# NVIDIA-Merlin/distributed-embeddings

Hardware: NVIDIA H100
Metric: DLRM global samples/sec (device-timed, max over ranks) (higher is better)
Workload: dtype bf16

## Files before the change

distributed_embeddings_b200/models/dlrm_fast.py:

```python
from __future__ import annotations

import os
from typing import Optional

import torch
from torch import nn

from ..ops import _native
from ..parallel.comm import CommContext
from ..parallel.fused import FusedEngine
from ..utils import nvtx
from ..utils.lr_schedule import LearningRateScheduler
from .dlrm import DLRM


def _pad8(n: int) -> int:
  return (n + 7) // 8 * 8


class _Layer:

  def __init__(self, lin: nn.Linear, relu: bool):
    self.lin = lin
    self.relu = relu
    self.out_f, self.in_f = lin.weight.shape
    self.in_pad = _pad8(self.in_f)
    self.w_off = self.b_off = 0
    self.w_numel = self.out_f * self.in_pad
    self.b_numel = _pad8(self.out_f)


class DLRMTrainStep:

  def __init__(self, model: DLRM, lr: float = 24.0, embedding_optimizer: str = "sgd",
               scheduler: Optional[LearningRateScheduler] = None, use_cuda_graph: bool = True,
               embedding_optimizer_kwargs: Optional[dict] = None, overlap: bool = True,
               gemm: str = "cublas"):
    if gemm not in ("cublas", "fused_dgrad", "tcgen05", "tcgen05_pair"):
      raise ValueError("gemm must be cublas | fused_dgrad | tcgen05 | tcgen05_pair")
    self.gemm = gemm
    self.model = model
    self.emb = model.embedding
    if self.emb.backend != "fused":
      raise ValueError("DLRMTrainStep needs the fused embedding back end")
    self.dev = self.emb.device
    self.ops = _native.require()
    self.world = self.emb.world_size
    self.ctx = CommContext.for_group(self.emb.group, self.dev)
    self.scheduler = scheduler
    self.use_cuda_graph = use_cuda_graph
    self.overlap = overlap
    self.emb.set_optimizer(embedding_optimizer, lr=lr, **(embedding_optimizer_kwargs or {}))
    if self.emb._engine is None:
      self.emb._engine = FusedEngine(self.emb)
    self.engine: FusedEngine = self.emb._engine
    self.n_emb = len(model.table_sizes)
    self.dim = model.embedding_dim
    sp_env = os.environ.get("DE_B200_STREAM_PUSH", "auto")
    self._stream_push = self.world > 1 and (sp_env == "1" or (sp_env == "auto" and self.world >= 4))
    self._push_stream = torch.cuda.Stream(device=self.dev) if self._stream_push else None
    self._push_ready = torch.cuda.Event() if self._stream_push else None

    lins_b = [m for m in model.bottom_mlp.net if isinstance(m, nn.Linear)]
    lins_t = [m for m in model.top_mlp.net if isinstance(m, nn.Linear)]
    self.bottom = [_Layer(l, True) for l in lins_b]
    self.top = [_Layer(l, True) for l in lins_t[:-1]]
    self.head = _Layer(lins_t[-1], False)
    if self.head.out_f != 1:
      raise ValueError("the top MLP must end in a single logit")
    layers = self.bottom + self.top + [self.head]
    self._dp_slots = []
    pos = 0
    if len(self.emb.dp_layers):
      if embedding_optimizer != "sgd":
        raise ValueError("replicated tables in the fast step are updated by the dense SGD "
                         "kernel: use embedding_optimizer='sgd' or data_parallel_threshold=None")
      for layer in self.emb.dp_layers:
        w = layer.embeddings
        self._dp_slots.append((pos, tuple(w.shape)))
        pos += _pad8(w.numel())
    for L in layers:
      L.w_off = pos
      pos += L.w_numel
      L.b_off = pos
      pos += L.b_numel
    self.n_flat = pos
    dev = self.dev
    self.p32 = torch.zeros(pos, dtype=torch.float32, device=dev)
    self.p16 = torch.zeros(pos, dtype=torch.bfloat16, device=dev)
    if self.world > 1:
      self.gsym = self.ctx.alloc_multicast(pos * 4, "dense_grads") or \
          self.ctx.alloc(pos * 4, "dense_grads")
      self.allreduce_kind = "nvls_multimem" if getattr(self.gsym, "mc_ptr", 0) else "p2p"
      self.g32 = self.gsym.view(torch.float32, (pos,))
    else:
      self.gsym = None
      self.allreduce_kind = "none"
      self.g32 = torch.zeros(pos, dtype=torch.float32, device=dev)
    with torch.no_grad():
      dp_targets = []
      for layer, (off, shape) in zip(self.emb.dp_layers, self._dp_slots):
        n = shape[0] * shape[1]
        view = self.p32[off:off + n].view(shape)
        view.copy_(layer.embeddings.data)
        layer.embeddings.data = view
        dp_targets.append(self.g32[off:off + n].view(shape))
      if self._dp_slots:
        self.engine.set_dp_grad_targets(dp_targets)
        self.engine._tables_dirty = True
        self.engine._key = None
      for L in layers:
        wv = self.p32[L.w_off:L.w_off + L.w_numel].view(L.out_f, L.in_pad)
        wv[:, :L.in_f].copy_(L.lin.weight)
        L.lin.weight.data = wv[:, :L.in_f]
        bv = self.p32[L.b_off:L.b_off + L.out_f]
        bv.copy_(L.lin.bias)
        L.lin.bias.data = bv
        L.w16 = self.p16[L.w_off:L.w_off + L.w_numel].view(L.out_f, L.in_pad)
        L.b16 = self.p16[L.b_off:L.b_off + L.out_f]
        L.gw = self.g32[L.w_off:L.w_off + L.w_numel].view(L.out_f, L.in_pad)
        L.gb = self.g32[L.b_off:L.b_off + L.b_numel]
        L.w16T = torch.empty(L.in_pad, L.out_f, dtype=torch.bfloat16, device=dev)
      self.p16.copy_(self.p32)
      self._refresh_transposes()
    self.lr_t = torch.full((1,), float(lr), dtype=torch.float32, device=dev)
    self.engine.share_lr(self.lr_t)
    self.lr = float(lr)
    self.loss = torch.zeros(1, dtype=torch.float32, device=dev)
    self._batch = None
    self._graph = None
    self._side = torch.cuda.Stream(device=dev) if overlap else None
    self._wgrad_overlap = os.environ.get("DE_B200_WGRAD_STREAM", "auto")
    self._wstream = torch.cuda.Stream(device=dev) if overlap else None
    ar_env = os.environ.get("DE_B200_AR_OVERLAP", "auto")
    ar_on = ar_env == "1" or (ar_env == "auto" and self.world >= 4)
    self._ar_stream = torch.cuda.Stream(device=dev) if (overlap and self.world > 1 and ar_on) \
        else None

  def _refresh_transposes(self):
    if self.gemm == "cublas":
      return
    for L in self.bottom[1:] + self.top[1:]:
      L.w16T.copy_(L.w16.t())

  def _linear_fwd(self, L, x):
    if self.gemm in ("tcgen05", "tcgen05_pair"):
      pair = self.gemm == "tcgen05_pair" and L.out_f >= 256
      self.ops.gemm_tn_bias_act(x, L.w16, L.b16, L.y, True, 512 if pair else 0)
    else:
      torch._addmm_activation(L.b16, x, L.w16.t(), out=L.y)
    return L.y

  def _wgrad(self, L, x):
    use = self._wstream is not None and (
        self._wgrad_overlap == "1" or
        (self._wgrad_overlap == "auto" and (self._batch or 0) >= 49152))
    if not use:
      torch.mm(L.dy.t(), x, out_dtype=torch.float32, out=L.gw)
      return
    self._w_used = True
    self._wstream.wait_stream(torch.cuda.current_stream())
    with torch.cuda.stream(self._wstream):
      torch.mm(L.dy.t(), x, out_dtype=torch.float32, out=L.gw)

  def _dgrad_relu(self, L, x_below, dx, gb_below):
    if self.gemm == "cublas":
      torch.mm(L.dy, L.w16, out=dx)
      self.ops.relu_bwd_bias(dx, x_below, gb_below)
    else:
      self.ops.gemm_dgrad_relu_bias(L.dy, L.w16T, x_below, dx, gb_below, 0)

  def _alloc(self, b: int):
    dev, bf = self.dev, torch.bfloat16
    if self._stream_push:
      self.engine.enable_streamed_push(max(1024, -(-b // 16)))
    self.engine.prepare(b, [1] * self.n_emb, ids64=False)
    self.cat_stage = self.engine.in_flat[:self.n_emb * b].view(self.n_emb, b)
    self.num_in = torch.zeros(b, self.bottom[0].in_f, dtype=torch.float32, device=dev)
    self.lab_in = torch.zeros(b, dtype=torch.float32, device=dev)
    self.x0 = torch.zeros(b, self.bottom[0].in_pad, dtype=bf, device=dev)
    for L in self.bottom + self.top:
      L.y = torch.empty(b, L.out_f, dtype=bf, device=dev)
      L.dy = torch.empty(b, L.out_f, dtype=bf, device=dev)
    self.z = torch.zeros(b, self.top[0].in_pad, dtype=bf, device=dev)
    self.dz = torch.empty(b, self.top[0].in_pad, dtype=bf, device=dev)
    self._batch = b
    self._graph = None
    self._stage = [(torch.zeros_like(self.cat_stage), torch.zeros_like(self.num_in),
                    torch.zeros_like(self.lab_in)) for _ in range(2)]
    self._slot_dev = torch.zeros(1, dtype=torch.int32, device=dev)
    self._slot_host = torch.tensor([[0], [1]], dtype=torch.int32).pin_memory()
    self._h2d_done = [torch.cuda.Event(), torch.cuda.Event()]
    self._consumed = [torch.cuda.Event(), torch.cuda.Event()]
    self._prefetched = 0
    self._consumed_n = 0
    self._use_stage = False

  def _forward(self):
    ops = self.ops
    if self._use_stage:
      a, b_ = self._stage
      ops.select_copy([a[0], a[1], a[2]], [b_[0], b_[1], b_[2]],
                      [self.cat_stage, self.num_in, self.lab_in], self._slot_dev)
    eng = self.engine
    if self._side is not None:
      self._side.wait_stream(torch.cuda.current_stream())
      with torch.cuda.stream(self._side):
        eng.launch_forward()
    ops.cast_pad(self.num_in, self.x0)
    x = self.x0
    for L in self.bottom:
      x = self._linear_fwd(L, x)
    if self._side is not None:
      torch.cuda.current_stream().wait_stream(self._side)
    else:
      eng.launch_forward()
    if eng.out_needs_reduce:
      eng.wait_output()
      ops.interact_fwd(x, eng.out, self.n_emb, self.z, [])
    else:
      ops.interact_fwd(x, eng.out, self.n_emb, self.z, eng.sync_out_wait())
    x = self.z
    for L in self.top:
      x = self._linear_fwd(L, x)

  def _backward(self):
    ops, eng = self.ops, self.engine
    b = self._batch
    last = self.top[-1]
    self.loss.zero_()
    H = self.head
    ops.head_loss(last.y, H.w16.view(-1), H.b16, self.lab_in, 1.0 / b, last.dy,
                  H.gw.view(-1), H.gb, last.gb, self.loss, None)
    for i in range(len(self.top) - 1, -1, -1):
      L = self.top[i]
      x = self.top[i - 1].y if i > 0 else self.z
      dx = self.top[i - 1].dy if i > 0 else self.dz
      self._wgrad(L, x)
      if i > 0:
        self._dgrad_relu(L, x, dx, self.top[i - 1].gb)
      else:
        torch.mm(L.dy, L.w16, out=dx)
    if self._ar_stream is not None:
      ar = self._ar_stream
      ar.wait_stream(torch.cuda.current_stream())
      if getattr(self, "_w_used", False):
        ar.wait_stream(self._wstream)
      off = self.top[0].w_off
      with torch.cuda.stream(ar):
        self.ctx.allreduce_(self.gsym, self.n_flat - off, torch.float32, scale=1.0 / self.world,
                            byte_offset=off * 4, max_blocks=32)
    hb = self.bottom[-1]
    pushed = eng.streamed_push
    if pushed:
      eng.push_counters.zero_()
      self._push_ready.record(torch.cuda.current_stream())
      ops.interact_bwd(hb.y, eng.out, self.n_emb, self.dz, hb.dy, 0, 0, 1.0, eng.routes_stage,
                       len(eng.routes_stage_np), [], eng.push_counters, eng.push_chunk_rows)
      self._push_stream.wait_event(self._push_ready)
      with torch.cuda.stream(self._push_stream):
        eng.launch_streamed_push()
    else:
      ops.interact_bwd(hb.y, eng.out, self.n_emb, self.dz, hb.dy, 0, 0, 1.0, eng.routes_all,
                       len(eng.routes_all_np), eng.sync_grad_signal(), None, 0)
    if self._side is not None:
      self._side.wait_stream(torch.cuda.current_stream())
      if pushed:
        self._side.wait_stream(self._push_stream)
      with torch.cuda.stream(self._side):
        eng.backward_inplace()
    else:
      if pushed:
        torch.cuda.current_stream().wait_stream(self._push_stream)
      eng.backward_inplace()
    ops.relu_bwd_bias(hb.dy, hb.y, hb.gb)
    for i in range(len(self.bottom) - 1, -1, -1):
      L = self.bottom[i]
      x = self.bottom[i - 1].y if i > 0 else self.x0
      self._wgrad(L, x)
      if i > 0:
        self._dgrad_relu(L, x, self.bottom[i - 1].dy, self.bottom[i - 1].gb)
    if self._dp_slots and self._side is not None:
      torch.cuda.current_stream().wait_stream(self._side)
    if getattr(self, "_w_used", False):
      torch.cuda.current_stream().wait_stream(self._wstream)
      self._w_used = False
    if self.world > 1:
      if self._ar_stream is not None:
        ar = self._ar_stream
        ar.wait_stream(torch.cuda.current_stream())
        with torch.cuda.stream(ar):
          self.ctx.allreduce_(self.gsym, self.top[0].w_off, torch.float32, scale=1.0 / self.world)
        torch.cuda.current_stream().wait_stream(ar)
      else:
        self.ctx.allreduce_(self.gsym, self.n_flat, torch.float32, scale=1.0 / self.world)
    ops.dense_sgd(self.p32, self.p16, self.g32, self.lr_t, 1.0)
    self._refresh_transposes()
    if self._side is not None:
      torch.cuda.current_stream().wait_stream(self._side)

  def _step_impl(self):
    with nvtx.range("dlrm_forward"):
      self._forward()
    with nvtx.range("dlrm_backward_update"):
      self._backward()

  def set_lr(self, lr: float):
    self.lr = float(lr)
    self.lr_t.fill_(self.lr)
    if self.emb._fused_optimizer is not None:
      self.emb._fused_optimizer["lr"] = self.lr

  def load_batch(self, numerical, categorical, labels):
    b = int(numerical.shape[0])
    if b != self._batch:
      self._alloc(b)
    self.num_in.copy_(numerical, non_blocking=True)
    self.lab_in.copy_(labels.reshape(-1), non_blocking=True)
    if isinstance(categorical, (list, tuple)):
      for v, c in zip(self.engine.in_views, categorical):
        v.copy_(c.reshape(v.shape), non_blocking=True)
    else:
      self.cat_stage.copy_(categorical, non_blocking=True)

  def prefetch(self, numerical, categorical, labels):
    b = int(numerical.shape[0])
    if b != self._batch:
      self._alloc(b)
    if not self._use_stage:
      self._use_stage = True
      self._graph = None
      self._copy_stream = torch.cuda.Stream(device=self.dev)
    slot = self._prefetched & 1
    cs = self._copy_stream
    if self._prefetched >= 2:
      cs.wait_event(self._consumed[slot])
    with torch.cuda.stream(cs):
      st = self._stage[slot]
      st[0].copy_(categorical, non_blocking=True)
      st[1].copy_(numerical, non_blocking=True)
      st[2].copy_(labels.reshape(-1), non_blocking=True)
      self._h2d_done[slot].record(cs)
    self._prefetched += 1

  def run_prefetched(self) -> torch.Tensor:
    assert self._consumed_n < self._prefetched, "call prefetch() first"
    slot = self._consumed_n & 1
    main = torch.cuda.current_stream()
    main.wait_event(self._h2d_done[slot])
    self._slot_dev.copy_(self._slot_host[slot], non_blocking=True)
    loss = self.run()
    self._consumed[slot].record(main)
    self._consumed_n += 1
    return loss

  def run(self) -> torch.Tensor:
    if self.scheduler is not None:
      self.set_lr(self.scheduler.step())
    if not self.use_cuda_graph:
      self._step_impl()
      return self.loss
    if self._graph is None:
      self.lr_t.zero_()
      self.engine.dry_updates(True)
      s = torch.cuda.Stream(device=self.dev)
      s.wait_stream(torch.cuda.current_stream())
      with torch.cuda.stream(s):
        for _ in range(2):
          self._step_impl()
      torch.cuda.current_stream().wait_stream(s)
      torch.cuda.synchronize()
      self.engine.dry_updates(False)
      g = torch.cuda.CUDAGraph()
      with torch.cuda.graph(g):
        self._step_impl()
      self._graph = g
      self.set_lr(self.lr)
    self._graph.replay()
    return self.loss

  def step(self, numerical, categorical, labels) -> torch.Tensor:
    self.load_batch(numerical, categorical, labels)
    return self.run()
```

distributed_embeddings_b200/ops/csrc/bindings.cpp:

```cpp
#include <ATen/cuda/CUDAContext.h>
#include <c10/cuda/CUDAGuard.h>
#include <c10/cuda/CUDAStream.h>
#include <cuda_runtime.h>
#include <torch/library.h>
#include <torch/torch.h>

#include <cstdlib>
#include <cstring>
#include <mutex>
#include <string>
#include <unordered_map>
#include <vector>

#include "de_b200.h"

namespace {

using at::Tensor;

#define DE_CUDA_CHECK(expr)                                                              \
  do {                                                                                   \
    cudaError_t _e = (expr);                                                             \
    TORCH_CHECK(_e == cudaSuccess, "CUDA error in " #expr ": ", cudaGetErrorString(_e)); \
  } while (0)

cudaStream_t cur_stream() { return at::cuda::getCurrentCUDAStream().stream(); }

int sm_count() {
  static int cached = -1;
  if (cached < 0) cached = at::cuda::getCurrentDeviceProperties()->multiProcessorCount;
  return cached;
}

de::PeerPtrs to_peers(at::IntArrayRef ptrs) {
  TORCH_CHECK(ptrs.size() <= de::kMaxPeers, "at most ", de::kMaxPeers, " peers are supported");
  de::PeerPtrs p;
  std::memset(&p, 0, sizeof(p));
  for (size_t i = 0; i < ptrs.size(); ++i) p.p[i] = reinterpret_cast<void*>(ptrs[i]);
  return p;
}

void check_launch() {
  cudaError_t e = cudaGetLastError();
  TORCH_CHECK(e == cudaSuccess, "kernel launch failed: ", cudaGetErrorString(e));
}

struct SyncCtx {
  de::PeerPtrs flags;
  uint32_t* state;
  int* error_flag;
  unsigned long long timeout;
  int rank, world;
};
std::vector<SyncCtx>& sync_ctxs() {
  static std::vector<SyncCtx> v;
  return v;
}
std::mutex& sync_mutex() {
  static std::mutex m;
  return m;
}

int64_t sync_ctx_create(at::IntArrayRef flag_ptrs, Tensor state, int64_t rank, int64_t world,
                        int64_t timeout_cycles, int64_t error_ptr) {
  TORCH_CHECK(state.is_cuda() && state.scalar_type() == at::kInt && state.is_contiguous() &&
                  state.numel() >= de::kSyncStateWords,
              "sync state must be an int32 CUDA tensor of >= ", de::kSyncStateWords, " words");
  SyncCtx c;
  c.flags = to_peers(flag_ptrs);
  c.state = reinterpret_cast<uint32_t*>(state.data_ptr<int>());
  c.error_flag = reinterpret_cast<int*>(error_ptr);
  c.timeout = static_cast<unsigned long long>(timeout_cycles);
  c.rank = static_cast<int>(rank);
  c.world = static_cast<int>(world);
  std::lock_guard<std::mutex> lock(sync_mutex());
  sync_ctxs().push_back(c);
  return static_cast<int64_t>(sync_ctxs().size()) - 1;
}

de::SyncArgs to_sync(at::IntArrayRef spec) {
  de::SyncArgs a = de::no_sync();
  if (spec.size() == 0) return a;
  TORCH_CHECK(spec.size() == 5, "sync spec = {handle, wait_ch, wait_abs_ch, signal_ch, slot}");
  SyncCtx c;
  {
    std::lock_guard<std::mutex> lock(sync_mutex());
    TORCH_CHECK(spec[0] >= 0 && spec[0] < static_cast<int64_t>(sync_ctxs().size()),
                "unknown sync context");
    c = sync_ctxs()[spec[0]];
  }
  for (int i = 1; i <= 3; ++i)
    TORCH_CHECK(spec[i] >= -1 && spec[i] < de::kSyncChannels, "sync channel out of range");
  TORCH_CHECK(spec[4] >= 0 && spec[4] < 2 * de::kSyncChannels, "sync counter slot out of range");
  a.flags = c.flags;
  a.state = c.state;
  a.error_flag = c.error_flag;
  a.timeout = c.timeout;
  a.rank = c.rank;
  a.world = c.world;
  a.wait_ch = static_cast<int32_t>(spec[1]);
  a.wait_abs_ch = static_cast<int32_t>(spec[2]);
  a.signal_ch = static_cast<int32_t>(spec[3]);
  a.counter_slot = static_cast<int32_t>(spec[4]);
  return a;
}

int dtype_code(at::ScalarType t) {
  if (t == at::kFloat) return 0;
  if (t == at::kBFloat16) return 1;
  if (t == at::kHalf) return 2;
  TORCH_CHECK(false, "activations / gradients must be fp32, bf16 or fp16");
  return -1;
}

void sync_only(at::IntArrayRef sync) {
  de::launch_sync_only(to_sync(sync), cur_stream());
  check_launch();
}

std::vector<int64_t> struct_sizes() {
  return {static_cast<int64_t>(sizeof(de::InputDesc)), static_cast<int64_t>(sizeof(de::TableDesc)),
          static_cast<int64_t>(de::kMaxPeers), static_cast<int64_t>(sizeof(de::GradRoute)),
          static_cast<int64_t>(de::kSyncStateWords)};
}

void lookup_fwd(const Tensor& descs, int64_t n_inputs, int64_t batch, int64_t src_batch,
                int64_t dst_batch, int64_t dst_stride, at::IntArrayRef src_ptrs,
                at::IntArrayRef dst_ptrs, int64_t rot, bool ids64, int64_t act_dtype, bool vec4,
                at::IntArrayRef sync, int64_t tile_samples, int64_t table_dtype, bool vec8) {
  TORCH_CHECK(descs.is_cuda(), "descs must live on the GPU");
  TORCH_CHECK(table_dtype >= 0 && table_dtype <= 2, "table_dtype: 0 fp32, 1 bf16, 2 fp16");
  c10::cuda::CUDAGuard guard(descs.device());
  de::launch_lookup_fwd(reinterpret_cast<const de::InputDesc*>(descs.data_ptr()),
                        static_cast<int>(n_inputs), batch, src_batch, dst_batch, dst_stride,
                        to_peers(src_ptrs), to_peers(dst_ptrs), static_cast<int>(rot), ids64,
                        static_cast<int>(act_dtype), vec4, sm_count(), cur_stream(),
                        to_sync(sync), static_cast<int>(tile_samples),
                        static_cast<int>(table_dtype), vec8);
  check_launch();
}

void scatter_add_bwd(const Tensor& descs, int64_t n_inputs, int64_t batch, int64_t src_batch,
                     int64_t grad_batch, int64_t grad_stride, at::IntArrayRef src_ptrs,
                     at::IntArrayRef grad_ptrs, int64_t rot, double scale, int64_t scale_ptr,
                     bool ids64, int64_t act_dtype, bool vec4, bool vec8, at::IntArrayRef sync,
                     bool staged) {
  TORCH_CHECK(descs.is_cuda(), "descs must live on the GPU");
  c10::cuda::CUDAGuard guard(descs.device());
  de::launch_scatter_add_bwd(reinterpret_cast<const de::InputDesc*>(descs.data_ptr()),
                             static_cast<int>(n_inputs), batch, src_batch, grad_batch, grad_stride,
                             to_peers(src_ptrs), to_peers(grad_ptrs), static_cast<int>(rot),
                             static_cast<float>(scale), reinterpret_cast<const float*>(scale_ptr),
                             ids64, static_cast<int>(act_dtype), vec4, sm_count(), cur_stream(),
                             vec8, to_sync(sync), staged);
  check_launch();
}

int bit_length(int64_t v) {
  int b = 0;
  while (v > 0) {
    ++b;
    v >>= 1;
  }
  return b < 1 ? 1 : b;
}

bool use_own_sort() {
  static const bool own = [] {
    const char* v = std::getenv("DE_B200_SORT");
    return !(v != nullptr && std::string(v) == "cub");
  }();
  return own;
}

std::tuple<Tensor, Tensor> radix_sort_pairs(const Tensor& keys, const Tensor& items,
                                            int64_t end_bit) {
  TORCH_CHECK(keys.is_cuda() && keys.scalar_type() == at::kLong && keys.is_contiguous());
  TORCH_CHECK(items.is_cuda() && items.scalar_type() == at::kInt && items.is_contiguous() &&
              items.numel() == keys.numel());
  c10::cuda::CUDAGuard guard(keys.device());
  const int64_t n = keys.numel();
  TORCH_CHECK(n < (int64_t(1) << 31), "own radix sort: too many items");
  Tensor ka = keys.clone(), ia = items.clone();
  Tensor kb = at::empty_like(ka), ib = at::empty_like(ia);
  if (n == 0) return {ka, ia};
  Tensor temp = at::empty({static_cast<int64_t>(de::radix_sort_temp_bytes(n))},
                          at::TensorOptions().device(keys.device()).dtype(at::kByte));
  int where = de::radix_sort_pairs(temp.data_ptr(), ka.data_ptr<int64_t>(),
                                   reinterpret_cast<uint32_t*>(ia.data_ptr<int>()),
                                   kb.data_ptr<int64_t>(),
                                   reinterpret_cast<uint32_t*>(ib.data_ptr<int>()), n,
                                   static_cast<int>(end_bit), cur_stream());
  check_launch();
  if (where == 0) return {ka, ia};
  return {kb, ib};
}

std::tuple<Tensor, Tensor> radix_sort_pairs32(const Tensor& keys, const Tensor& items,
                                              int64_t end_bit) {
  TORCH_CHECK(keys.is_cuda() && keys.scalar_type() == at::kInt && keys.is_contiguous());
  TORCH_CHECK(items.is_cuda() && items.scalar_type() == at::kInt && items.is_contiguous() &&
              items.numel() == keys.numel());
  c10::cuda::CUDAGuard guard(keys.device());
  const int64_t n = keys.numel();
  TORCH_CHECK(n < (int64_t(1) << 31), "own radix sort: too many items");
  Tensor ka = keys.clone(), ia = items.clone();
  Tensor kb = at::empty_like(ka), ib = at::empty_like(ia);
  Tensor out = at::empty({n}, keys.options().dtype(at::kLong));
  if (n == 0) return {out, ia};
  Tensor temp = at::empty({static_cast<int64_t>(de::radix_sort_temp_bytes(n))},
                          at::TensorOptions().device(keys.device()).dtype(at::kByte));
  int where = de::radix_sort_pairs32(
      temp.data_ptr(), reinterpret_cast<uint32_t*>(ka.data_ptr<int>()),
      reinterpret_cast<uint32_t*>(ia.data_ptr<int>()),
      reinterpret_cast<uint32_t*>(kb.data_ptr<int>()),
      reinterpret_cast<uint32_t*>(ib.data_ptr<int>()), out.data_ptr<int64_t>(), n,
      static_cast<int>(end_bit), cur_stream());
  check_launch();
  return {out, where == 0 ? ia : ib};
}

std::tuple<Tensor, Tensor> head_segments(const Tensor& sorted_keys) {
  TORCH_CHECK(sorted_keys.is_cuda() && sorted_keys.scalar_type() == at::kLong &&
              sorted_keys.is_contiguous());
  c10::cuda::CUDAGuard guard(sorted_keys.device());
  const int64_t n = sorted_keys.numel();
  auto i64 = at::TensorOptions().device(sorted_keys.device()).dtype(at::kLong);
  Tensor seg_start = at::empty({n + 1}, i64);
  Tensor n_unique = at::zeros({1}, i64);
  if (n == 0) return {seg_start, n_unique};
  Tensor temp = at::empty({static_cast<int64_t>(de::head_segments_temp_bytes(n))},
                          at::TensorOptions().device(sorted_keys.device()).dtype(at::kByte));
  de::head_segments(temp.data_ptr(), sorted_keys.data_ptr<int64_t>(), n,
                    seg_start.data_ptr<int64_t>(), n_unique.data_ptr<int64_t>(), cur_stream());
  check_launch();
  return {seg_start, n_unique};
}

std::tuple<Tensor, Tensor, Tensor, Tensor> sort_items(const Tensor& descs, const Tensor& tables,
                                                      int64_t n_tables, int64_t n_inputs,
                                                      int64_t batch, int64_t src_batch,
                                                      at::IntArrayRef src_ptrs, bool ids64,
                                                      int64_t n_items, int64_t total_rows,
                                                      bool prefill_sentinel) {
  TORCH_CHECK(descs.is_cuda() && tables.is_cuda());
  TORCH_CHECK(n_inputs * batch < (int64_t(1) << 32),
              "sorted update: n_inputs * batch = ", n_inputs * batch, " does not fit 32-bit items");
  c10::cuda::CUDAGuard guard(descs.device());
  auto stream = cur_stream();
  auto i64 = at::TensorOptions().device(descs.device()).dtype(at::kLong);
  auto i32 = at::TensorOptions().device(descs.device()).dtype(at::kInt);
  Tensor keys = prefill_sentinel ? at::full({n_items}, total_rows, i64) : at::empty({n_items}, i64);
  Tensor keys_sorted = at::empty({n_items}, i64);
  Tensor items = at::empty({n_items}, i32), items_sorted = at::empty({n_items}, i32);
  Tensor seg_start = at::empty({n_items + 1}, i64);
  Tensor n_unique = at::zeros({1}, i64);
  if (n_items == 0) return {keys_sorted, items_sorted, seg_start, n_unique};
  if (use_own_sort() && total_rows < (int64_t(1) << 32) - 1) {
    TORCH_CHECK(n_items < (int64_t(1) << 31), "own radix sort: too many items");
    Tensor k32a = prefill_sentinel
                      ? at::full({n_items}, static_cast<int64_t>(static_cast<int32_t>(
                                                static_cast<uint32_t>(total_rows))), i32)
                      : at::empty({n_items}, i32);
    Tensor k32b = at::empty({n_items}, i32);
    de::launch_build_keys(reinterpret_cast<const de::InputDesc*>(descs.data_ptr()),
                          reinterpret_cast<const de::TableDesc*>(tables.data_ptr()),
                          static_cast<int>(n_tables), static_cast<int>(n_inputs), batch,
                          src_batch, to_peers(src_ptrs), ids64, k32a.data_ptr(),
                          reinterpret_cast<uint32_t*>(items.data_ptr<int>()), sm_count(), stream,
                          true);
    check_launch();
    size_t sort_bytes = de::radix_sort_temp_bytes(n_items);
    size_t head_bytes = de::head_segments_temp_bytes(n_items);
    Tensor temp = at::empty({static_cast<int64_t>(std::max(sort_bytes, head_bytes))},
                            at::TensorOptions().device(descs.device()).dtype(at::kByte));
    int where = de::radix_sort_pairs32(
        temp.data_ptr(), reinterpret_cast<uint32_t*>(k32a.data_ptr<int>()),
        reinterpret_cast<uint32_t*>(items.data_ptr<int>()),
        reinterpret_cast<uint32_t*>(k32b.data_ptr<int>()),
        reinterpret_cast<uint32_t*>(items_sorted.data_ptr<int>()),
        keys_sorted.data_ptr<int64_t>(), n_items, bit_length(total_rows), stream);
    if (where == 0) std::swap(items, items_sorted);
    de::head_segments(temp.data_ptr(), keys_sorted.data_ptr<int64_t>(), n_items,
                      seg_start.data_ptr<int64_t>(), n_unique.data_ptr<int64_t>(), stream);
    check_launch();
    return {keys_sorted, items_sorted, seg_start, n_unique};
  }
  de::launch_build_keys(reinterpret_cast<const de::InputDesc*>(descs.data_ptr()),
                        reinterpret_cast<const de::TableDesc*>(tables.data_ptr()),
                        static_cast<int>(n_tables), static_cast<int>(n_inputs), batch, src_batch,
                        to_peers(src_ptrs), ids64, keys.data_ptr<int64_t>(),
                        reinterpret_cast<uint32_t*>(items.data_ptr<int>()), sm_count(), stream);
  check_launch();
  if (use_own_sort()) {
    TORCH_CHECK(n_items < (int64_t(1) << 31), "own radix sort: too many items");
    size_t sort_bytes = de::radix_sort_temp_bytes(n_items);
    size_t head_bytes = de::head_segments_temp_bytes(n_items);
    Tensor temp = at::empty({static_cast<int64_t>(std::max(sort_bytes, head_bytes))},
                            at::TensorOptions().device(descs.device()).dtype(at::kByte));
    int where = de::radix_sort_pairs(temp.data_ptr(), keys.data_ptr<int64_t>(),
                                     reinterpret_cast<uint32_t*>(items.data_ptr<int>()),
                                     keys_sorted.data_ptr<int64_t>(),
                                     reinterpret_cast<uint32_t*>(items_sorted.data_ptr<int>()),
                                     n_items, bit_length(total_rows), stream);
    if (where == 0) {
      std::swap(keys, keys_sorted);
      std::swap(items, items_sorted);
    }
    de::head_segments(temp.data_ptr(), keys_sorted.data_ptr<int64_t>(), n_items,
                      seg_start.data_ptr<int64_t>(), n_unique.data_ptr<int64_t>(), stream);
    check_launch();
    return {keys_sorted, items_sorted, seg_start, n_unique};
  }
  size_t sort_bytes = de::sort_pairs_temp_bytes(n_items);
  size_t uniq_bytes = de::unique_temp_bytes(n_items);
  Tensor temp = at::empty({static_cast<int64_t>(std::max(sort_bytes, uniq_bytes)) + 16},
                          at::TensorOptions().device(descs.device()).dtype(at::kByte));
  de::sort_pairs(temp.data_ptr(), sort_bytes, keys.data_ptr<int64_t>(),
                 keys_sorted.data_ptr<int64_t>(),
                 reinterpret_cast<const uint32_t*>(items.data_ptr<int>()),
                 reinterpret_cast<uint32_t*>(items_sorted.data_ptr<int>()), n_items,
                 bit_length(total_rows), stream);
  de::unique_segments(temp.data_ptr(), uniq_bytes, keys_sorted.data_ptr<int64_t>(), n_items,
                      seg_start.data_ptr<int64_t>(), n_unique.data_ptr<int64_t>(), stream);
  check_launch();
  return {keys_sorted, items_sorted, seg_start, n_unique};
}

void segment_update(const Tensor& descs, const Tensor& tables, int64_t n_tables, int64_t batch,
                    int64_t grad_batch, int64_t grad_stride, at::IntArrayRef grad_ptrs,
                    const Tensor& sorted_keys, const Tensor& sorted_items, const Tensor& seg_start,
                    const Tensor& n_unique, int64_t opt_kind, double lr, double eps, double beta1,
                    double beta2, double bias1, double bias2, double grad_scale,
                    double weight_decay, int64_t lr_ptr, const c10::optional<Tensor>& emit_keys,
                    const c10::optional<Tensor>& emit_rows, int64_t max_width, int64_t act_dtype,
                    bool vec4, const c10::optional<Tensor>& scratch, int64_t step_ptr,
                    int64_t table_dtype) {
  c10::cuda::CUDAGuard guard(descs.device());
  TORCH_CHECK(table_dtype >= 0 && table_dtype <= 2, "table_dtype: 0 fp32, 1 bf16, 2 fp16");
  de::OptimizerArgs opt;
  opt.kind = static_cast<int32_t>(opt_kind);
  opt.lr = static_cast<float>(lr);
  opt.eps = static_cast<float>(eps);
  opt.beta1 = static_cast<float>(beta1);
  opt.beta2 = static_cast<float>(beta2);
  opt.bias1 = static_cast<float>(bias1);
  opt.bias2 = static_cast<float>(bias2);
  opt.grad_scale = static_cast<float>(grad_scale);
  opt.weight_decay = static_cast<float>(weight_decay);
  opt.lr_ptr = reinterpret_cast<const float*>(lr_ptr);
  opt.step_ptr = reinterpret_cast<const float*>(step_ptr);
  if (opt.kind == de::kOptEmit) TORCH_CHECK(emit_keys.has_value() && emit_rows.has_value());
  if (scratch.has_value() && vec4 && max_width <= 128 && opt.kind != de::kOptEmit) {
    const int64_t n_items = sorted_keys.numel();
    const int64_t sw = (max_width + 3) / 4 * 4;
    TORCH_CHECK(scratch->scalar_type() == at::kFloat && scratch->is_contiguous() &&
                    scratch->numel() >= ((n_items + 31) / 32) * sw,
                "scratch too small for the balanced update");
    bool ok = de::launch_balanced_update(
        reinterpret_cast<const de::InputDesc*>(descs.data_ptr()),
        reinterpret_cast<const de::TableDesc*>(tables.data_ptr()), static_cast<int>(n_tables),
        batch, grad_batch, grad_stride, to_peers(grad_ptrs), sorted_keys.data_ptr<int64_t>(),
        reinterpret_cast<const uint32_t*>(sorted_items.data_ptr<int>()), n_items,
        seg_start.data_ptr<int64_t>(), n_unique.data_ptr<int64_t>(), opt,
        scratch->data_ptr<float>(), static_cast<int>(sw), static_cast<int>(max_width),
        static_cast<int>(act_dtype), sm_count(), cur_stream(), static_cast<int>(table_dtype));
    TORCH_CHECK(ok, "balanced update launch failed");
    check_launch();
    return;
  }
  de::launch_segment_update(
      reinterpret_cast<const de::InputDesc*>(descs.data_ptr()),
      reinterpret_cast<const de::TableDesc*>(tables.data_ptr()), static_cast<int>(n_tables), batch,
      grad_batch, grad_stride, to_peers(grad_ptrs), sorted_keys.data_ptr<int64_t>(),
      reinterpret_cast<const uint32_t*>(sorted_items.data_ptr<int>()),
      seg_start.data_ptr<int64_t>(), n_unique.data_ptr<int64_t>(), sorted_keys.numel(), opt,
      emit_keys.has_value() ? emit_keys->data_ptr<int64_t>() : nullptr,
      emit_rows.has_value() ? emit_rows->data_ptr<float>() : nullptr, static_cast<int>(max_width),
      static_cast<int>(act_dtype), vec4, sm_count(), cur_stream(), static_cast<int>(table_dtype));
  check_launch();
}

Tensor upload_bytes(const void* host, size_t bytes, const at::Device& dev) {
  Tensor t = at::empty({static_cast<int64_t>(bytes)},
                       at::TensorOptions().device(dev).dtype(at::kByte));
  DE_CUDA_CHECK(cudaMemcpyAsync(t.data_ptr(), host, bytes, cudaMemcpyHostToDevice, cur_stream()));
  return t;
}

de::InputDesc single_desc(const void* table, const Tensor& values,
                          const c10::optional<Tensor>& offsets, int64_t hotness, int64_t rows,
                          int64_t width, int64_t combiner) {
  de::InputDesc d;
  std::memset(&d, 0, sizeof(d));
  d.table = table;
  d.ids = values.data_ptr();
  d.offsets = offsets.has_value() ? offsets->data_ptr<int64_t>() : nullptr;
  d.sub_rows = rows;
  d.width = static_cast<int32_t>(width);
  d.hotness = offsets.has_value() ? 0 : static_cast<int32_t>(hotness);
  d.combiner = static_cast<int32_t>(combiner);
  return d;
}

void check_ids(const Tensor& values, const c10::optional<Tensor>& offsets) {
  TORCH_CHECK(values.is_cuda() && values.is_contiguous(), "ids must be a contiguous CUDA tensor");
  TORCH_CHECK(values.scalar_type() == at::kInt || values.scalar_type() == at::kLong,
              "ids must be int32 or int64");
  if (offsets.has_value())
    TORCH_CHECK(offsets->is_cuda() && offsets->scalar_type() == at::kLong &&
                    offsets->is_contiguous(),
                "row_splits must be a contiguous int64 CUDA tensor");
}

Tensor embedding_lookup_fwd(const Tensor& param, const Tensor& values,
                            const c10::optional<Tensor>& offsets, int64_t hotness, int64_t batch,
                            int64_t combiner, bool out_bf16) {
  const auto pt = param.scalar_type();
  TORCH_CHECK(param.is_cuda() && param.dim() == 2 &&
                  (pt == at::kFloat || pt == at::kBFloat16 || pt == at::kHalf) &&
                  param.is_contiguous(),
              "param must be a contiguous fp32, bf16 or fp16 [rows, width] CUDA tensor");
  check_ids(values, offsets);
  c10::cuda::CUDAGuard guard(param.device());
  const int64_t width = param.size(1);
  const int tdt = dtype_code(pt);
  Tensor out = at::empty({batch, width}, param.options().dtype(out_bf16 ? at::kBFloat16 : pt));
  if (batch == 0) return out;
  de::InputDesc d = single_desc(param.data_ptr(), values, offsets, hotness, param.size(0), width,
                                combiner);
  Tensor dd = upload_bytes(&d, sizeof(d), param.device());
  de::PeerPtrs src, dst;
  std::memset(&src, 0, sizeof(src));
  std::memset(&dst, 0, sizeof(dst));
  dst.p[0] = out.data_ptr();
  const int64_t avg_hot = std::max<int64_t>(1, values.numel() / std::max<int64_t>(batch, 1));
  int64_t lanes_per_row = 1;
  while (lanes_per_row < (width + 3) / 4 && lanes_per_row < 32) lanes_per_row *= 2;
  const int64_t ts = std::max<int64_t>(32 / lanes_per_row, std::min<int64_t>(32, 64 / avg_hot));
  de::launch_lookup_fwd(reinterpret_cast<const de::InputDesc*>(dd.data_ptr()), 1, batch, batch,
                        batch, width, src, dst, 0, values.scalar_type() == at::kLong,
                        out_bf16 ? 1 : tdt, width % 4 == 0, sm_count(), cur_stream(),
                        de::no_sync(), static_cast<int>(std::max<int64_t>(1, ts)), tdt,
                        width % 8 == 0 && reinterpret_cast<uintptr_t>(param.data_ptr()) % 16 == 0);
  check_launch();
  return out;
}

void embedding_scatter_add(Tensor dst, const Tensor& values, const c10::optional<Tensor>& offsets,
                           int64_t hotness, int64_t batch, int64_t combiner, const Tensor& grad,
                           double scale) {
  TORCH_CHECK(dst.is_cuda() && dst.dim() == 2 && dst.scalar_type() == at::kFloat &&
              dst.is_contiguous());
  TORCH_CHECK(grad.is_cuda() && grad.dim() == 2 && grad.stride(1) == 1);
  check_ids(values, offsets);
  if (batch == 0) return;
  c10::cuda::CUDAGuard guard(dst.device());
  const int64_t width = dst.size(1);
  de::InputDesc d = single_desc(dst.data_ptr(), values, offsets, hotness, dst.size(0), width,
                                combiner);
  Tensor dd = upload_bytes(&d, sizeof(d), dst.device());
  de::PeerPtrs src, gp;
  std::memset(&src, 0, sizeof(src));
  std::memset(&gp, 0, sizeof(gp));
  gp.p[0] = grad.data_ptr();
  const int gdt = dtype_code(grad.scalar_type());
  const int64_t gstride = grad.stride(0);
  const bool vec4 = (width % 4 == 0) && (gstride % 4 == 0) &&
                    (reinterpret_cast<uintptr_t>(grad.data_ptr()) % 16 == 0);
  de::launch_scatter_add_bwd(reinterpret_cast<const de::InputDesc*>(dd.data_ptr()), 1, batch,
                             batch, batch, gstride, src, gp, 0, static_cast<float>(scale), nullptr,
                             values.scalar_type() == at::kLong, gdt, vec4, sm_count(),
                             cur_stream(), false, de::no_sync());
  check_launch();
}

std::tuple<Tensor, Tensor> embedding_lookup_grad(const Tensor& values,
                                                 const c10::optional<Tensor>& offsets,
                                                 int64_t hotness, int64_t batch, int64_t combiner,
                                                 const Tensor& grad, int64_t num_rows) {
  TORCH_CHECK(grad.is_cuda() && grad.dim() == 2 && grad.stride(1) == 1);
  check_ids(values, offsets);
  c10::cuda::CUDAGuard guard(grad.device());
  const int64_t width = grad.size(1);
  const int64_t n_items = values.numel();
  auto f32 = grad.options().dtype(at::kFloat);
  auto i64 = grad.options().dtype(at::kLong);
  if (n_items == 0) return {at::empty({0}, i64), at::empty({0, width}, f32)};
  de::InputDesc d = single_desc(nullptr, values, offsets, hotness, num_rows, width, combiner);
  de::TableDesc t;
  std::memset(&t, 0, sizeof(t));
  t.rows = num_rows;
  t.width = static_cast<int32_t>(width);
  Tensor dd = upload_bytes(&d, sizeof(d), grad.device());
  Tensor td = upload_bytes(&t, sizeof(t), grad.device());
  auto sorted = sort_items(dd, td, 1, 1, batch, batch, {}, values.scalar_type() == at::kLong,
                           n_items, num_rows, false);
  Tensor emit_keys = at::empty({n_items}, i64);
  Tensor emit_rows = at::empty({n_items, width}, f32);
  const int gdt = dtype_code(grad.scalar_type());
  const int64_t gstride = grad.stride(0);
  const bool vec4 = (width % 4 == 0) && (gstride % 4 == 0) &&
                    (reinterpret_cast<uintptr_t>(grad.data_ptr()) % 16 == 0);
  std::vector<int64_t> gp = {reinterpret_cast<int64_t>(grad.data_ptr())};
  segment_update(dd, td, 1, batch, batch, gstride, gp, std::get<0>(sorted), std::get<1>(sorted),
                 std::get<2>(sorted), std::get<3>(sorted), de::kOptEmit, 0, 0, 0, 0, 1, 1, 1.0, 0, 0,
                 emit_keys, emit_rows, width, gdt, vec4, c10::nullopt, 0, 0);
  int64_t n_unique = std::get<3>(sorted).item<int64_t>();
  if (n_unique > 0) {
    int64_t last = emit_keys.narrow(0, n_unique - 1, 1).item<int64_t>();
    if (last >= num_rows) --n_unique;
  }
  return {emit_keys.narrow(0, 0, n_unique), emit_rows.narrow(0, 0, n_unique)};
}

Tensor row_to_split(const Tensor& indices, int64_t num_rows) {
  TORCH_CHECK(indices.is_cuda() && indices.dim() == 2 && indices.size(1) == 2 &&
                  indices.scalar_type() == at::kLong && indices.is_contiguous(),
              "indices must be a contiguous int64 [nnz, 2] CUDA tensor");
  c10::cuda::CUDAGuard guard(indices.device());
  Tensor splits = at::empty({num_rows + 1}, indices.options());
  de::launch_row_to_split(indices.data_ptr<int64_t>(), indices.size(0), num_rows,
                          splits.data_ptr<int64_t>(), cur_stream());
  check_launch();
  return splits;
}

void hash_init(Tensor table) {
  TORCH_CHECK(table.is_cuda() && table.scalar_type() == at::kLong && table.is_contiguous());
  c10::cuda::CUDAGuard guard(table.device());
  de::launch_hash_init(table.data_ptr<int64_t>(), table.numel() / 2, cur_stream());
  check_launch();
}

Tensor integer_lookup(Tensor table, Tensor count, Tensor next_index, const Tensor& keys,
                      int64_t capacity) {
  TORCH_CHECK(table.is_cuda() && count.is_cuda() && next_index.is_cuda() && keys.is_cuda());
  TORCH_CHECK(table.scalar_type() == at::kLong && keys.scalar_type() == at::kLong &&
              next_index.scalar_type() == at::kLong && count.scalar_type() == at::kInt);
  c10::cuda::CUDAGuard guard(table.device());
  Tensor k = keys.contiguous();
  Tensor out = at::empty_like(k);
  de::launch_integer_lookup(table.data_ptr<int64_t>(), table.numel() / 2,
                            reinterpret_cast<uint32_t*>(count.data_ptr<int>()),
                            next_index.data_ptr<int64_t>(), k.data_ptr<int64_t>(), k.numel(),
                            capacity, out.data_ptr<int64_t>(), cur_stream());
  check_launch();
  return out;
}

void barrier(at::IntArrayRef flag_ptrs, Tensor epoch, int64_t rank, int64_t world, int64_t channel,
             int64_t timeout_cycles, int64_t error_ptr) {
  c10::cuda::CUDAGuard guard(epoch.device());
  de::launch_barrier(to_peers(flag_ptrs), reinterpret_cast<uint32_t*>(epoch.data_ptr<int>()),
                     static_cast<int>(rank), static_cast<int>(world), static_cast<int>(channel),
                     static_cast<unsigned long long>(timeout_cycles),
                     reinterpret_cast<int*>(error_ptr), cur_stream());
  check_launch();
}

void allreduce(at::IntArrayRef buf_ptrs, at::IntArrayRef flag_ptrs, Tensor epoch, int64_t rank,
               int64_t world, int64_t n_elems, double scale, bool bf16, int64_t channel,
               int64_t timeout_cycles, int64_t error_ptr, int64_t mc_ptr, int64_t max_blocks) {
  c10::cuda::CUDAGuard guard(epoch.device());
  if (mc_ptr != 0) {
    de::launch_allreduce_multimem(reinterpret_cast<void*>(mc_ptr), to_peers(flag_ptrs),
                                  reinterpret_cast<uint32_t*>(epoch.data_ptr<int>()),
                                  static_cast<int>(rank), static_cast<int>(world), n_elems,
                                  static_cast<float>(scale), bf16, static_cast<int>(channel),
                                  static_cast<unsigned long long>(timeout_cycles),
                                  reinterpret_cast<int*>(error_ptr), sm_count(), cur_stream(),
                         static_cast<int>(max_blocks));
  } else {
    de::launch_allreduce(to_peers(buf_ptrs), to_peers(flag_ptrs),
                         reinterpret_cast<uint32_t*>(epoch.data_ptr<int>()),
                         static_cast<int>(rank), static_cast<int>(world), n_elems,
                         static_cast<float>(scale), bf16, static_cast<int>(channel),
                         static_cast<unsigned long long>(timeout_cycles),
                         reinterpret_cast<int*>(error_ptr), sm_count(), cur_stream(),
                         static_cast<int>(max_blocks));
  }
  check_launch();
}

void p2p_store_bench(const Tensor& src, int64_t dst_ptr, int64_t n_rows, int64_t row_bytes,
                     int64_t vec_bytes, int64_t dst_stride, int64_t unroll, int64_t blocks,
                     int64_t threads) {
  TORCH_CHECK(src.is_cuda() && src.is_contiguous() &&
              src.numel() * src.element_size() >= n_rows * row_bytes);
  TORCH_CHECK(row_bytes % vec_bytes == 0 && (vec_bytes == 4 || vec_bytes == 8 || vec_bytes == 16));
  TORCH_CHECK((row_bytes / vec_bytes >= 32 && (row_bytes / vec_bytes) % 32 == 0) ||
              32 % (row_bytes / vec_bytes) == 0);
  TORCH_CHECK(unroll >= 1 && unroll <= 8 && threads % 32 == 0 && threads <= 1024);
  c10::cuda::CUDAGuard guard(src.device());
  de::launch_p2p_store_bench(src.data_ptr(), reinterpret_cast<void*>(dst_ptr), n_rows,
                             static_cast<int>(row_bytes), static_cast<int>(vec_bytes), dst_stride,
                             static_cast<int>(unroll), static_cast<int>(blocks),
                             static_cast<int>(threads), cur_stream());
  check_launch();
}

void push_segments(const Tensor& segs, const Tensor& src, at::IntArrayRef dst_ptrs,
                   int64_t max_seg_elems, at::IntArrayRef sync) {
  TORCH_CHECK(segs.is_cuda() && segs.scalar_type() == at::kLong && segs.is_contiguous() &&
              segs.dim() == 2 && segs.size(1) == 4);
  TORCH_CHECK(src.is_cuda() && src.is_contiguous() &&
              (src.element_size() == 4 || src.element_size() == 8));
  c10::cuda::CUDAGuard guard(src.device());
  de::launch_push_segments(segs.data_ptr<int64_t>(), static_cast<int>(segs.size(0)),
                           src.data_ptr(), to_peers(dst_ptrs),
                           static_cast<int>(src.element_size()), max_seg_elems, sm_count(),
                           cur_stream(), to_sync(sync));
  check_launch();
}

void push_grad(const Tensor& routes, int64_t n_routes, const Tensor& src, int64_t dst_dtype,
               double scale, at::IntArrayRef sync) {
  TORCH_CHECK(routes.is_cuda() && routes.scalar_type() == at::kByte &&
              routes.numel() >= n_routes * static_cast<int64_t>(sizeof(de::GradRoute)));
  TORCH_CHECK(src.is_cuda() && src.dim() == 2 && src.stride(1) == 1);
  c10::cuda::CUDAGuard guard(src.device());
  de::launch_push_grad(reinterpret_cast<const de::GradRoute*>(routes.data_ptr()),
                       static_cast<int>(n_routes), src.data_ptr(), src.stride(0),
                       dtype_code(src.scalar_type()), static_cast<int>(dst_dtype), src.size(0),
                       static_cast<float>(scale), sm_count(), cur_stream(), to_sync(sync));
  check_launch();
}

void stream_push(at::IntArrayRef src_ptrs, at::IntArrayRef dst_ptrs, at::IntArrayRef row_bytes,
                 const Tensor& counters, int64_t chunk_rows, int64_t rows, int64_t blocks,
                 at::IntArrayRef sync) {
  TORCH_CHECK(src_ptrs.size() == dst_ptrs.size() && src_ptrs.size() == row_bytes.size() &&
              src_ptrs.size() <= de::kMaxPeers);
  TORCH_CHECK(counters.is_cuda() && counters.scalar_type() == at::kInt && chunk_rows > 0 &&
              counters.numel() >= (rows + chunk_rows - 1) / chunk_rows);
  de::PushPlan plan;
  std::memset(&plan, 0, sizeof(plan));
  plan.n = static_cast<int32_t>(src_ptrs.size());
  for (size_t i = 0; i < src_ptrs.size(); ++i) {
    TORCH_CHECK(row_bytes[i] % 16 == 0 && src_ptrs[i] % 16 == 0 && dst_ptrs[i] % 16 == 0,
                "streamed push needs 16-byte aligned rows");
    plan.src[i] = reinterpret_cast<const void*>(src_ptrs[i]);
    plan.dst[i] = reinterpret_cast<void*>(dst_ptrs[i]);
    plan.row_bytes[i] = row_bytes[i];
  }
  c10::cuda::CUDAGuard guard(counters.device());
  de::SyncArgs sa = to_sync(sync);
  de::launch_stream_push(plan, reinterpret_cast<const uint32_t*>(counters.data_ptr<int>()),
                         static_cast<int>(chunk_rows), rows, sa.timeout, sa.error_flag,
                         static_cast<int>(blocks), cur_stream(), sa);
  check_launch();
}

void rowslice_reduce(const Tensor& partial, int64_t out_ptr, int64_t out_stride,
                     int64_t out_dtype, const Tensor& cols) {
  TORCH_CHECK(partial.is_cuda() && partial.dim() == 3 && partial.scalar_type() == at::kFloat &&
              partial.is_contiguous());
  TORCH_CHECK(cols.is_cuda() && cols.scalar_type() == at::kInt && cols.is_contiguous() &&
              cols.dim() == 2 && cols.size(1) == 3);
  c10::cuda::CUDAGuard guard(partial.device());
  de::launch_rowslice_reduce(partial.data_ptr<float>(), static_cast<int>(partial.size(0)),
                             partial.size(1), partial.size(2), reinterpret_cast<void*>(out_ptr),
                             out_stride, static_cast<int>(out_dtype), cols.data_ptr<int>(),
                             static_cast<int>(cols.size(0)), cur_stream());
  check_launch();
}

void gather_segments(const Tensor& segs, at::IntArrayRef src_ptrs, Tensor dst,
                     int64_t max_seg_elems) {
  TORCH_CHECK(segs.is_cuda() && segs.scalar_type() == at::kLong && segs.is_contiguous());
  TORCH_CHECK(dst.is_cuda() && dst.is_contiguous());
  c10::cuda::CUDAGuard guard(dst.device());
  de::launch_gather_segments(segs.data_ptr<int64_t>(), static_cast<int>(segs.size(0)),
                             to_peers(src_ptrs), dst.data_ptr(),
                             static_cast<int>(dst.element_size()), max_seg_elems, cur_stream());
  check_launch();
}

void gather_ragged(const Tensor& segs, at::IntArrayRef val_ptrs, at::IntArrayRef split_ptrs,
                   Tensor dst_vals, Tensor goff, int64_t b, int64_t max_cap) {
  TORCH_CHECK(segs.is_cuda() && segs.scalar_type() == at::kLong && segs.is_contiguous());
  TORCH_CHECK(goff.is_cuda() && goff.scalar_type() == at::kLong && dst_vals.is_cuda());
  c10::cuda::CUDAGuard guard(dst_vals.device());
  de::launch_gather_ragged(segs.data_ptr<int64_t>(), static_cast<int>(segs.size(0)),
                           to_peers(val_ptrs), to_peers(split_ptrs), dst_vals.data_ptr(),
                           goff.data_ptr<int64_t>(), b, static_cast<int>(val_ptrs.size()),
                           static_cast<int>(dst_vals.element_size()), max_cap, cur_stream());
  check_launch();
}

void select_copy(at::TensorList src0, at::TensorList src1, at::TensorList dst,
                 const Tensor& slot_flag) {
  TORCH_CHECK(src0.size() == dst.size() && src1.size() == dst.size() && dst.size() <= 4);
  TORCH_CHECK(slot_flag.is_cuda() && slot_flag.scalar_type() == at::kInt);
  const void* s0[4];
  const void* s1[4];
  void* d[4];
  int64_t nb[4];
  for (size_t i = 0; i < dst.size(); ++i) {
    TORCH_CHECK(src0[i].is_contiguous() && src1[i].is_contiguous() && dst[i].is_contiguous());
    nb[i] = dst[i].numel() * dst[i].element_size();
    TORCH_CHECK(src0[i].numel() * src0[i].element_size() == nb[i] &&
                src1[i].numel() * src1[i].element_size() == nb[i] && nb[i] % 16 == 0,
                "select_copy segments must match and be multiples of 16 bytes");
    s0[i] = src0[i].data_ptr();
    s1[i] = src1[i].data_ptr();
    d[i] = dst[i].data_ptr();
  }
  c10::cuda::CUDAGuard guard(slot_flag.device());
  de::launch_select_copy(s0, s1, d, nb, static_cast<int>(dst.size()), slot_flag.data_ptr<int>(),
                         sm_count(), cur_stream());
  check_launch();
}

void copy_cast_2d(const Tensor& src, int64_t dst_ptr, int64_t dst_stride, int64_t dst_dtype,
                  double scale) {
  TORCH_CHECK(src.is_cuda() && src.dim() == 2 && src.stride(1) == 1);
  c10::cuda::CUDAGuard guard(src.device());
  de::launch_copy_cast_2d(src.data_ptr(), src.stride(0), reinterpret_cast<void*>(dst_ptr),
                          dst_stride, src.size(0), src.size(1), dtype_code(src.scalar_type()),
                          static_cast<int>(dst_dtype), static_cast<float>(scale), cur_stream());
  check_launch();
}

void check_bf16_2d(const Tensor& t, const char* name) {
  TORCH_CHECK(t.is_cuda() && t.dim() == 2 && t.scalar_type() == at::kBFloat16 && t.stride(1) == 1,
              name, " must be a 2-D bf16 CUDA tensor with unit inner stride");
}

void interact_fwd(const Tensor& bottom, const Tensor& emb, int64_t n_emb, Tensor z,
                  at::IntArrayRef sync) {
  check_bf16_2d(bottom, "bottom");
  check_bf16_2d(emb, "emb");
  check_bf16_2d(z, "z");
  c10::cuda::CUDAGuard guard(bottom.device());
  const int64_t dim = bottom.size(1);
  TORCH_CHECK(emb.size(1) == n_emb * dim);
  const int64_t need = (n_emb + 1) * n_emb / 2 + dim;
  TORCH_CHECK(z.size(1) >= need, "z is too narrow");
  bool ok = de::launch_interact_fwd(bottom.data_ptr(), bottom.stride(0), emb.data_ptr(),
                                    emb.stride(0), static_cast<int>(n_emb), static_cast<int>(dim),
                                    z.data_ptr(), z.stride(0), static_cast<int>(z.size(1)),
                                    bottom.size(0), sm_count(), cur_stream(), to_sync(sync));
  TORCH_CHECK(ok, "unsupported interaction shape (n_emb <= 31, dim in {16,32,64,128})");
  check_launch();
}

void interact_bwd(const Tensor& bottom, const Tensor& emb, int64_t n_emb, const Tensor& dz,
                  Tensor dbottom, int64_t demb_ptr, int64_t demb_stride, double emb_grad_scale,
                  const c10::optional<Tensor>& routes, int64_t n_routes, at::IntArrayRef sync,
                  const c10::optional<Tensor>& done_counters, int64_t chunk_rows) {
  check_bf16_2d(bottom, "bottom");
  check_bf16_2d(emb, "emb");
  check_bf16_2d(dz, "dz");
  check_bf16_2d(dbottom, "dbottom");
  if (routes.has_value())
    TORCH_CHECK(routes->is_cuda() && routes->scalar_type() == at::kByte &&
                routes->numel() >= n_routes * static_cast<int64_t>(sizeof(de::GradRoute)));
  c10::cuda::CUDAGuard guard(bottom.device());
  const int64_t dim = bottom.size(1);
  bool ok = de::launch_interact_bwd(bottom.data_ptr(), bottom.stride(0), emb.data_ptr(),
                                    emb.stride(0), static_cast<int>(n_emb), static_cast<int>(dim),
                                    dz.data_ptr(), dz.stride(0), dbottom.data_ptr(),
                                    dbottom.stride(0), reinterpret_cast<void*>(demb_ptr),
                                    demb_stride, static_cast<float>(emb_grad_scale),
                                    bottom.size(0), sm_count(), cur_stream(),
                                    routes.has_value()
                                        ? reinterpret_cast<const de::GradRoute*>(routes->data_ptr())
                                        : nullptr,
                                    static_cast<int>(n_routes), to_sync(sync),
                                    done_counters.has_value()
                                        ? reinterpret_cast<uint32_t*>(done_counters->data_ptr<int>())
                                        : nullptr,
                                    static_cast<int>(chunk_rows));
  TORCH_CHECK(ok, "unsupported interaction shape (n_emb <= 31, dim in {32,64,128}; routed / "
                  "signalling launches need dim in {64,128} and 16-byte aligned rows)");
  check_launch();
}

void avgpool_fwd(const Tensor& x, int64_t n, Tensor out, int64_t stride) {
  check_bf16_2d(x, "x");
  check_bf16_2d(out, "out");
  const int64_t out_len = (n + stride - 1) / stride;
  TORCH_CHECK(x.size(1) >= n && out.size(1) >= out_len && out.size(0) == x.size(0));
  const int64_t pad = std::max<int64_t>(0, (out_len - 1) * stride + stride - n);
  c10::cuda::CUDAGuard guard(x.device());
  de::launch_avgpool_fwd(x.data_ptr(), x.stride(0), static_cast<int>(n), out.data_ptr(),
                         out.stride(0), static_cast<int>(out_len), static_cast<int>(stride),
                         static_cast<int>(pad / 2), x.size(0), cur_stream());
  check_launch();
}

void avgpool_bwd(const Tensor& dout, Tensor dx, int64_t n, int64_t stride) {
  check_bf16_2d(dout, "dout");
  check_bf16_2d(dx, "dx");
  const int64_t out_len = (n + stride - 1) / stride;
  TORCH_CHECK(dx.size(1) >= n && dout.size(1) >= out_len && dout.size(0) == dx.size(0));
  const int64_t pad = std::max<int64_t>(0, (out_len - 1) * stride + stride - n);
  c10::cuda::CUDAGuard guard(dx.device());
  de::launch_avgpool_bwd(dout.data_ptr(), dout.stride(0), static_cast<int>(out_len),
                         dx.data_ptr(), dx.stride(0), static_cast<int>(n),
                         static_cast<int>(stride), static_cast<int>(pad / 2), dx.size(0),
                         cur_stream());
  check_launch();
}

void relu_bwd_bias(Tensor dy, const Tensor& y, Tensor db) {
  check_bf16_2d(dy, "dy");
  check_bf16_2d(y, "y");
  TORCH_CHECK(dy.is_contiguous() && y.is_contiguous() && dy.size(1) % 8 == 0);
  TORCH_CHECK(db.is_cuda() && db.scalar_type() == at::kFloat && db.numel() >= dy.size(1));
  c10::cuda::CUDAGuard guard(dy.device());
  de::launch_relu_bwd_bias(dy.data_ptr(), y.data_ptr(), db.data_ptr<float>(), dy.size(0),
                           static_cast<int>(dy.size(1)), cur_stream());
  check_launch();
}

void head_loss(const Tensor& x, const Tensor& w, const Tensor& bias, const Tensor& labels,
               double inv_batch, Tensor dx, Tensor dw, Tensor db, Tensor dbias_prev,
               Tensor loss_sum, const c10::optional<Tensor>& logits) {
  check_bf16_2d(x, "x");
  TORCH_CHECK(x.is_contiguous() && dx.is_contiguous());
  TORCH_CHECK(w.scalar_type() == at::kBFloat16 && bias.scalar_type() == at::kBFloat16);
  TORCH_CHECK(labels.scalar_type() == at::kFloat && labels.is_contiguous());
  c10::cuda::CUDAGuard guard(x.device());
  bool ok = de::launch_head_loss(x.data_ptr(), static_cast<int>(x.size(1)), w.data_ptr(),
                                 bias.data_ptr(), labels.data_ptr<float>(), x.size(0),
                                 static_cast<float>(inv_batch), dx.data_ptr(),
                                 dw.data_ptr<float>(), db.data_ptr<float>(),
                                 dbias_prev.data_ptr<float>(), loss_sum.data_ptr<float>(),
                                 logits.has_value() ? logits->data_ptr<float>() : nullptr,
                                 sm_count(), cur_stream());
  TORCH_CHECK(ok, "head_loss supports K in {64,128,256,512,1024}");
  check_launch();
}

void dense_sgd(Tensor p32, Tensor p16, Tensor g32, const Tensor& lr, double grad_scale) {
  TORCH_CHECK(p32.is_cuda() && p32.scalar_type() == at::kFloat && g32.scalar_type() == at::kFloat &&
              p16.scalar_type() == at::kBFloat16 && lr.scalar_type() == at::kFloat);
  TORCH_CHECK(p32.numel() % 4 == 0 && p32.numel() == g32.numel() && p32.numel() == p16.numel());
  c10::cuda::CUDAGuard guard(p32.device());
  de::launch_sgd_update(p32.data_ptr<float>(), p16.data_ptr(), g32.data_ptr<float>(),
                        lr.data_ptr<float>(), static_cast<float>(grad_scale), p32.numel(),
                        sm_count(), cur_stream());
  check_launch();
}

void cast_pad(const Tensor& src, Tensor dst) {
  TORCH_CHECK(src.is_cuda() && src.scalar_type() == at::kFloat && src.is_contiguous());
  TORCH_CHECK(dst.scalar_type() == at::kBFloat16 && dst.is_contiguous() &&
              dst.size(0) == src.size(0) && dst.size(1) >= src.size(1));
  c10::cuda::CUDAGuard guard(src.device());
  de::launch_cast_pad(src.data_ptr<float>(), static_cast<int>(src.size(1)), dst.data_ptr(),
                      static_cast<int>(dst.size(1)), src.size(0), cur_stream());
  check_launch();
}

void gemm_tn_bias_act(const Tensor& a, const Tensor& b, const c10::optional<Tensor>& bias,
                      Tensor out, bool relu, int64_t block_n) {
  check_bf16_2d(a, "a");
  check_bf16_2d(b, "b");
  check_bf16_2d(out, "out");
  TORCH_CHECK(a.size(1) == b.size(1) && out.size(0) == a.size(0) && out.size(1) == b.size(0),
              "shape mismatch");
  if (bias.has_value())
    TORCH_CHECK(bias->is_cuda() && bias->scalar_type() == at::kBFloat16 && bias->is_contiguous() &&
                bias->numel() == b.size(0));
  c10::cuda::CUDAGuard guard(a.device());
  bool ok = de::launch_gemm_tn_bias_act(
      a.data_ptr(), a.stride(0), b.data_ptr(), b.stride(0),
      bias.has_value() ? bias->data_ptr() : nullptr, out.data_ptr(), out.stride(0),
      static_cast<int>(a.size(0)), static_cast<int>(b.size(0)), static_cast<int>(a.size(1)), relu,
      static_cast<int>(block_n), sm_count(), cur_stream());
  TORCH_CHECK(ok, "gemm_tn_bias_act: unsupported shape/alignment or launch failure");
  check_launch();
}

void gemm_dgrad_relu_bias(const Tensor& dy, const Tensor& wt, const Tensor& act, Tensor dx,
                          Tensor colsum, int64_t block_n) {
  check_bf16_2d(dy, "dy");
  check_bf16_2d(wt, "wt");
  check_bf16_2d(act, "act");
  check_bf16_2d(dx, "dx");
  TORCH_CHECK(dy.size(1) == wt.size(1) && dx.size(0) == dy.size(0) && dx.size(1) == wt.size(0) &&
              act.size(0) == dx.size(0) && act.size(1) == dx.size(1), "shape mismatch");
  TORCH_CHECK(colsum.is_cuda() && colsum.scalar_type() == at::kFloat &&
              colsum.numel() >= dx.size(1));
  c10::cuda::CUDAGuard guard(dy.device());
  bool ok = de::launch_gemm_tn_fused(
      dy.data_ptr(), dy.stride(0), wt.data_ptr(), wt.stride(0), nullptr, dx.data_ptr(),
      dx.stride(0), static_cast<int>(dy.size(0)), static_cast<int>(wt.size(0)),
      static_cast<int>(dy.size(1)), 2, act.data_ptr(), act.stride(0), colsum.data_ptr<float>(),
      static_cast<int>(block_n), sm_count(), cur_stream());
  TORCH_CHECK(ok, "gemm_dgrad_relu_bias: unsupported shape/alignment or launch failure");
  check_launch();
}

Tensor symm_alloc(int64_t nbytes, int64_t device_index) {
  c10::cuda::CUDAGuard guard(static_cast<c10::DeviceIndex>(device_index));
  void* ptr = nullptr;
  const size_t padded = (static_cast<size_t>(nbytes) + 255) & ~static_cast<size_t>(255);
  DE_CUDA_CHECK(cudaMalloc(&ptr, padded));
  DE_CUDA_CHECK(cudaMemset(ptr, 0, padded));
  DE_CUDA_CHECK(cudaDeviceSynchronize());
  auto deleter = [](void* p) { cudaFree(p); };
  return at::from_blob(ptr, {static_cast<int64_t>(padded)}, deleter,
                       at::TensorOptions()
                           .device(at::Device(at::kCUDA, static_cast<c10::DeviceIndex>(device_index)))
                           .dtype(at::kByte));
}

Tensor ipc_get_handle(const Tensor& buf) {
  TORCH_CHECK(buf.is_cuda());
  cudaIpcMemHandle_t h;
  DE_CUDA_CHECK(cudaIpcGetMemHandle(&h, buf.data_ptr()));
  Tensor out = at::empty({static_cast<int64_t>(sizeof(h))}, at::TensorOptions().dtype(at::kByte));
  std::memcpy(out.data_ptr(), &h, sizeof(h));
  return out;
}

int64_t ipc_open(const Tensor& handle, int64_t device_index) {
  TORCH_CHECK(!handle.is_cuda() && handle.numel() == sizeof(cudaIpcMemHandle_t));
  c10::cuda::CUDAGuard guard(static_cast<c10::DeviceIndex>(device_index));
  cudaIpcMemHandle_t h;
  std::memcpy(&h, handle.data_ptr(), sizeof(h));
  void* ptr = nullptr;
  DE_CUDA_CHECK(cudaIpcOpenMemHandle(&ptr, h, cudaIpcMemLazyEnablePeerAccess));
  return reinterpret_cast<int64_t>(ptr);
}

void ipc_close(int64_t ptr, int64_t device_index) {
  c10::cuda::CUDAGuard guard(static_cast<c10::DeviceIndex>(device_index));
  cudaIpcCloseMemHandle(reinterpret_cast<void*>(ptr));
}

int64_t host_device_pointer(const Tensor& host) {
  TORCH_CHECK(!host.is_cuda());
  void* dptr = nullptr;
  DE_CUDA_CHECK(cudaHostGetDevicePointer(&dptr, host.data_ptr(), 0));
  return reinterpret_cast<int64_t>(dptr);
}

}

TORCH_LIBRARY(de_b200, m) {
  m.def("struct_sizes() -> int[]", &struct_sizes);
  m.def(
      "sync_ctx_create(int[] flag_ptrs, Tensor state, int rank, int world, int timeout_cycles, "
      "int error_ptr) -> int",
      &sync_ctx_create);
  m.def("sync_only(int[] sync) -> ()", &sync_only);
  m.def(
      "lookup_fwd(Tensor descs, int n_inputs, int batch, int src_batch, int dst_batch, "
      "int dst_stride, int[] src_ptrs, int[] dst_ptrs, int rot, bool ids64, int act_dtype, "
      "bool vec4, int[] sync, int tile_samples, int table_dtype=0, bool vec8=False) -> ()",
      &lookup_fwd);
  m.def(
      "scatter_add_bwd(Tensor descs, int n_inputs, int batch, int src_batch, int grad_batch, "
      "int grad_stride, int[] src_ptrs, int[] grad_ptrs, int rot, float scale, int scale_ptr, bool ids64, "
      "int act_dtype, bool vec4, bool vec8, int[] sync, bool staged) -> ()",
      &scatter_add_bwd);
  m.def(
      "sort_items(Tensor descs, Tensor tables, int n_tables, int n_inputs, int batch, "
      "int src_batch, int[] src_ptrs, bool ids64, int n_items, int total_rows, "
      "bool prefill_sentinel) -> "
      "(Tensor, Tensor, Tensor, Tensor)",
      &sort_items);
  m.def("radix_sort_pairs(Tensor keys, Tensor items, int end_bit) -> (Tensor, Tensor)",
        &radix_sort_pairs);
  m.def("radix_sort_pairs32(Tensor keys, Tensor items, int end_bit) -> (Tensor, Tensor)",
        &radix_sort_pairs32);
  m.def("head_segments(Tensor sorted_keys) -> (Tensor, Tensor)", &head_segments);
  m.def(
      "segment_update(Tensor descs, Tensor tables, int n_tables, int batch, int grad_batch, "
      "int grad_stride, int[] grad_ptrs, Tensor sorted_keys, Tensor sorted_items, "
      "Tensor seg_start, Tensor n_unique, int opt_kind, float lr, float eps, float beta1, "
      "float beta2, float bias1, float bias2, float grad_scale, float weight_decay, int lr_ptr, "
      "Tensor? emit_keys, Tensor? emit_rows, int max_width, int act_dtype, bool vec4, "
      "Tensor? scratch, int step_ptr, int table_dtype=0) -> ()",
      &segment_update);
  m.def(
      "embedding_lookup_fwd(Tensor param, Tensor values, Tensor? offsets, int hotness, int batch, "
      "int combiner, bool out_bf16) -> Tensor",
      &embedding_lookup_fwd);
  m.def(
      "embedding_scatter_add(Tensor(a!) dst, Tensor values, Tensor? offsets, int hotness, "
      "int batch, int combiner, Tensor grad, float scale) -> ()",
      &embedding_scatter_add);
  m.def(
      "embedding_lookup_grad(Tensor values, Tensor? offsets, int hotness, int batch, int combiner, "
      "Tensor grad, int num_rows) -> (Tensor, Tensor)",
      &embedding_lookup_grad);
  m.def("row_to_split(Tensor indices, int num_rows) -> Tensor", &row_to_split);
  m.def("hash_init(Tensor(a!) table) -> ()", &hash_init);
  m.def(
      "integer_lookup(Tensor(a!) table, Tensor(b!) count, Tensor(c!) next_index, Tensor keys, "
      "int capacity) -> Tensor",
      &integer_lookup);
  m.def(
      "barrier(int[] flag_ptrs, Tensor(a!) epoch, int rank, int world, int channel, "
      "int timeout_cycles, int error_ptr) -> ()",
      &barrier);
  m.def(
      "allreduce(int[] buf_ptrs, int[] flag_ptrs, Tensor(a!) epoch, int rank, int world, "
      "int n_elems, float scale, bool bf16, int channel, int timeout_cycles, "
      "int error_ptr, int mc_ptr, int max_blocks) -> ()",
      &allreduce);
  m.def("gather_segments(Tensor segs, int[] src_ptrs, Tensor(a!) dst, int max_seg_elems) -> ()",
        &gather_segments);
  m.def(
      "p2p_store_bench(Tensor src, int dst_ptr, int n_rows, int row_bytes, int vec_bytes, "
      "int dst_stride, int unroll, int blocks, int threads) -> ()",
      &p2p_store_bench);
  m.def(
      "push_segments(Tensor segs, Tensor src, int[] dst_ptrs, int max_seg_elems, int[] sync) -> ()",
      &push_segments);
  m.def(
      "push_grad(Tensor routes, int n_routes, Tensor src, int dst_dtype, float scale, int[] sync) "
      "-> ()",
      &push_grad);
  m.def(
      "stream_push(int[] src_ptrs, int[] dst_ptrs, int[] row_bytes, Tensor counters, "
      "int chunk_rows, int rows, int blocks, int[] sync) -> ()",
      &stream_push);
  m.def(
      "rowslice_reduce(Tensor partial, int out_ptr, int out_stride, int out_dtype, Tensor cols) "
      "-> ()",
      &rowslice_reduce);
  m.def(
      "gather_ragged(Tensor segs, int[] val_ptrs, int[] split_ptrs, Tensor(a!) dst_vals, "
      "Tensor(b!) goff, int b, int max_cap) -> ()",
      &gather_ragged);
  m.def("select_copy(Tensor[] src0, Tensor[] src1, Tensor(a!)[] dst, Tensor slot_flag) -> ()",
        &select_copy);
  m.def("copy_cast_2d(Tensor src, int dst_ptr, int dst_stride, int dst_dtype, float scale) -> ()",
        &copy_cast_2d);
  m.def("interact_fwd(Tensor bottom, Tensor emb, int n_emb, Tensor(a!) z, int[] sync) -> ()",
        &interact_fwd);
  m.def(
      "interact_bwd(Tensor bottom, Tensor emb, int n_emb, Tensor dz, Tensor(a!) dbottom, "
      "int demb_ptr, int demb_stride, float emb_grad_scale, Tensor? routes, int n_routes, "
      "int[] sync, Tensor? done_counters, int chunk_rows) -> ()",
      &interact_bwd);
  m.def("avgpool_fwd(Tensor x, int n, Tensor(a!) out, int stride) -> ()", &avgpool_fwd);
  m.def("avgpool_bwd(Tensor dout, Tensor(a!) dx, int n, int stride) -> ()", &avgpool_bwd);
  m.def("relu_bwd_bias(Tensor(a!) dy, Tensor y, Tensor(b!) db) -> ()", &relu_bwd_bias);
  m.def(
      "head_loss(Tensor x, Tensor w, Tensor bias, Tensor labels, float inv_batch, Tensor(a!) dx, "
      "Tensor(b!) dw, Tensor(c!) db, Tensor(d!) dbias_prev, Tensor(e!) loss_sum, Tensor? logits) "
      "-> ()",
      &head_loss);
  m.def(
      "dense_sgd(Tensor(a!) p32, Tensor(b!) p16, Tensor(c!) g32, Tensor lr, float grad_scale) "
      "-> ()",
      &dense_sgd);
  m.def("cast_pad(Tensor src, Tensor(a!) dst) -> ()", &cast_pad);
  m.def(
      "gemm_tn_bias_act(Tensor a, Tensor b, Tensor? bias, Tensor(a!) out, bool relu, int block_n) "
      "-> ()",
      &gemm_tn_bias_act);
  m.def(
      "gemm_dgrad_relu_bias(Tensor dy, Tensor wt, Tensor act, Tensor(a!) dx, Tensor(b!) colsum, "
      "int block_n) -> ()",
      &gemm_dgrad_relu_bias);
  m.def("symm_alloc(int nbytes, int device_index) -> Tensor", &symm_alloc);
  m.def("ipc_get_handle(Tensor buf) -> Tensor", &ipc_get_handle);
  m.def("ipc_open(Tensor handle, int device_index) -> int", &ipc_open);
  m.def("ipc_close(int ptr, int device_index) -> ()", &ipc_close);
  m.def("host_device_pointer(Tensor host) -> int", &host_device_pointer);
}
```

distributed_embeddings_b200/ops/csrc/de_b200.h:

```cpp
#pragma once
#include <cuda_runtime.h>
#include <stdint.h>

namespace de {

constexpr int kMaxPeers = 16;
constexpr int kGridCapSms = 132;

struct alignas(16) InputDesc {
  const void* table;
  const void* ids;
  const int64_t* offsets;
  int64_t ids_off;
  int64_t id_shift;
  int64_t sub_rows;
  int64_t row_base;
  int32_t width;
  int32_t hotness;
  int32_t dst_col;
  int32_t combiner;
  int32_t local_table;
  int32_t flags;
  int64_t item_off;
};

struct PeerPtrs {
  void* p[kMaxPeers];
};

constexpr int kSyncChannels = 16;
constexpr int kSyncStateWords = 64;
struct SyncArgs {
  PeerPtrs flags;
  uint32_t* state;
  int* error_flag;
  unsigned long long timeout;
  int32_t rank, world;
  int32_t wait_ch;
  int32_t wait_abs_ch;
  int32_t signal_ch;
  int32_t counter_slot;
};
inline SyncArgs no_sync() {
  SyncArgs s{};
  s.state = nullptr;
  s.wait_ch = s.wait_abs_ch = s.signal_ch = -1;
  return s;
}

struct alignas(16) GradRoute {
  void* dst;
  int64_t dst_stride;
  int32_t src_col;
  int32_t width;
  int32_t dst_col;
  int32_t pad;
};

enum OptimizerKind : int32_t { kOptSGD = 0, kOptAdagrad = 1, kOptRowwiseAdagrad = 2, kOptAdam = 3, kOptEmit = 4 };

struct alignas(16) TableDesc {
  void* weight;
  void* state0;
  void* state1;
  int64_t rows;
  int64_t key_base;
  int32_t width;
  int32_t pad;
};

struct OptimizerArgs {
  int32_t kind;
  float lr;
  float eps;
  float beta1, beta2;
  float bias1, bias2;
  float grad_scale;
  float weight_decay;
  const float* lr_ptr;
  const float* step_ptr;
};

void launch_lookup_fwd(const InputDesc* descs, int n_inputs, int64_t batch, int64_t src_batch,
                       int64_t dst_batch, int64_t dst_stride, const PeerPtrs& src,
                       const PeerPtrs& dst, int rot, bool ids64, int act_dtype, bool vec4,
                       int sm_count, cudaStream_t stream, const SyncArgs& sync,
                       int tile_samples = 32, int table_dtype = 0, bool vec8 = false);

void launch_scatter_add_bwd(const InputDesc* descs, int n_inputs, int64_t batch, int64_t src_batch,
                            int64_t grad_batch, int64_t grad_stride, const PeerPtrs& src,
                            const PeerPtrs& grad, int rot, float scale, const float* scale_ptr,
                            bool ids64, int act_dtype, bool vec4, int sm_count,
                            cudaStream_t stream, bool vec8, const SyncArgs& sync,
                            bool staged = false);

void launch_build_keys(const InputDesc* descs, const TableDesc* tables, int n_tables, int n_inputs,
                       int64_t batch, int64_t src_batch, const PeerPtrs& src, bool ids64, void* keys,
                       uint32_t* items, int sm_count, cudaStream_t stream, bool keys32 = false);
size_t sort_pairs_temp_bytes(int64_t n);
void sort_pairs(void* temp, size_t temp_bytes, const int64_t* keys_in, int64_t* keys_out,
                const uint32_t* items_in, uint32_t* items_out, int64_t n, int end_bit,
                cudaStream_t stream);
size_t unique_temp_bytes(int64_t n);
void unique_segments(void* temp, size_t temp_bytes, const int64_t* sorted_keys, int64_t n,
                     int64_t* seg_start, int64_t* n_unique, cudaStream_t stream);
size_t radix_sort_temp_bytes(int64_t n);
int radix_sort_pairs(void* temp, int64_t* keys_a, uint32_t* items_a, int64_t* keys_b,
                     uint32_t* items_b, int64_t n, int end_bit, cudaStream_t stream);
int radix_sort_pairs32(void* temp, uint32_t* keys_a, uint32_t* items_a, uint32_t* keys_b,
                       uint32_t* items_b, int64_t* keys_out64, int64_t n, int end_bit,
                       cudaStream_t stream);
size_t head_segments_temp_bytes(int64_t n);
void head_segments(void* temp, const int64_t* sorted_keys, int64_t n, int64_t* seg_start,
                   int64_t* n_unique, cudaStream_t stream);
void launch_segment_update(const InputDesc* descs, const TableDesc* tables, int n_tables,
                           int64_t batch, int64_t grad_batch, int64_t grad_stride,
                           const PeerPtrs& grad, const int64_t* sorted_keys,
                           const uint32_t* sorted_items, const int64_t* seg_start,
                           const int64_t* n_unique, int64_t n_items, const OptimizerArgs& opt,
                           int64_t* emit_keys, float* emit_rows, int max_width, int act_dtype,
                           bool vec4, int sm_count, cudaStream_t stream, int table_dtype = 0);

bool launch_balanced_update(const InputDesc* descs, const TableDesc* tables, int n_tables,
                            int64_t batch, int64_t grad_batch, int64_t grad_stride,
                            const PeerPtrs& grad, const int64_t* sorted_keys,
                            const uint32_t* sorted_items, int64_t n_items,
                            const int64_t* seg_start, const int64_t* n_unique,
                            const OptimizerArgs& opt, float* scratch, int scratch_width,
                            int max_width, int act_dtype, int sm_count, cudaStream_t stream,
                            int table_dtype = 0);

void launch_row_to_split(const int64_t* coo_indices, int64_t nnz, int64_t num_rows,
                         int64_t* row_splits, cudaStream_t stream);
void launch_hash_init(int64_t* table, int64_t n_slots, cudaStream_t stream);
void launch_integer_lookup(int64_t* table, int64_t n_slots, uint32_t* counts, int64_t* next_index,
                           const int64_t* keys, int64_t n, int64_t capacity, int64_t* out,
                           cudaStream_t stream);

void launch_barrier(const PeerPtrs& flags, uint32_t* epoch, int rank, int world, int channel,
                    unsigned long long timeout_cycles, int* error_flag, cudaStream_t stream);
void launch_allreduce(const PeerPtrs& bufs, const PeerPtrs& flags, uint32_t* epoch, int rank,
                      int world, int64_t n_elems, float scale, bool bf16, int channel,
                      unsigned long long timeout_cycles, int* error_flag, int sm_count,
                      cudaStream_t stream, int max_blocks = 0);
void launch_allreduce_multimem(void* mc_ptr, const PeerPtrs& flags, uint32_t* epoch, int rank,
                               int world, int64_t n_elems, float scale, bool bf16, int channel,
                               unsigned long long timeout_cycles, int* error_flag, int sm_count,
                               cudaStream_t stream, int max_blocks = 0);
void launch_p2p_store_bench(const void* src, void* dst, int64_t n_rows, int row_bytes,
                            int vec_bytes, int64_t dst_stride, int unroll, int blocks, int threads,
                            cudaStream_t stream);
void launch_sync_only(const SyncArgs& sync, cudaStream_t stream);
void launch_push_segments(const int64_t* segs, int n_seg, const void* src, const PeerPtrs& dst,
                          int elem_bytes, int64_t max_seg_elems, int sm_count,
                          cudaStream_t stream, const SyncArgs& sync);
void launch_push_grad(const GradRoute* routes, int n_routes, const void* src, int64_t src_stride,
                      int src_dtype, int dst_dtype, int64_t rows, float scale, int sm_count,
                      cudaStream_t stream, const SyncArgs& sync);
struct PushPlan {
  const void* src[kMaxPeers];
  void* dst[kMaxPeers];
  int64_t row_bytes[kMaxPeers];
  int32_t n;
};
void launch_stream_push(const PushPlan& plan, const uint32_t* counters, int chunk_rows,
                        int64_t rows, unsigned long long timeout, int* error_flag, int blocks,
                        cudaStream_t stream, const SyncArgs& sync);
void launch_rowslice_reduce(const float* partial, int world, int64_t rows, int64_t part_stride,
                            void* out, int64_t out_stride, int out_dtype, const int32_t* cols,
                            int n_cols, cudaStream_t stream);
void launch_gather_segments(const int64_t* segs, int n_seg, const PeerPtrs& src, void* dst,
                            int elem_bytes, int64_t max_seg_elems, cudaStream_t stream);
void launch_gather_ragged(const int64_t* segs, int n_seg, const PeerPtrs& src_vals,
                          const PeerPtrs& src_splits, void* dst_vals, int64_t* goff, int64_t b,
                          int world, int elem_bytes, int64_t max_cap, cudaStream_t stream);
void launch_select_copy(const void* const* src0, const void* const* src1, void* const* dst,
                        const int64_t* nbytes, int count, const int* slot_flag, int sm_count,
                        cudaStream_t stream);
void launch_copy_cast_2d(const void* src, int64_t src_stride, void* dst, int64_t dst_stride,
                         int64_t rows, int64_t cols, int src_dtype, int dst_dtype, float scale,
                         cudaStream_t stream);

bool launch_interact_fwd(const void* bottom, int64_t bottom_stride, const void* emb,
                         int64_t emb_stride, int n_emb, int dim, void* z, int64_t z_stride,
                         int z_width, int64_t batch, int sm_count, cudaStream_t stream,
                         const SyncArgs& sync);
bool launch_interact_bwd(const void* bottom, int64_t bottom_stride, const void* emb,
                         int64_t emb_stride, int n_emb, int dim, const void* dz,
                         int64_t dz_stride, void* dbottom, int64_t dbottom_stride, void* demb,
                         int64_t demb_stride, float emb_grad_scale, int64_t batch, int sm_count,
                         cudaStream_t stream, const GradRoute* routes, int n_routes,
                         const SyncArgs& sync, uint32_t* done_counters = nullptr,
                         int chunk_rows = 0);
void launch_avgpool_fwd(const void* x, int64_t x_stride, int n, void* out, int64_t out_stride,
                        int out_len, int stride, int left, int64_t rows, cudaStream_t stream);
void launch_avgpool_bwd(const void* dout, int64_t dout_stride, int out_len, void* dx,
                        int64_t dx_stride, int n, int stride, int left, int64_t rows,
                        cudaStream_t stream);
void launch_relu_bwd_bias(void* dy, const void* y, float* db, int64_t rows, int cols,
                          cudaStream_t stream);
bool launch_head_loss(const void* x, int K, const void* w, const void* bias, const float* labels,
                      int64_t batch, float inv_batch, void* dx, float* dw, float* db,
                      float* dbias_prev, float* loss_sum, float* logits_out, int sm_count,
                      cudaStream_t stream);
void launch_sgd_update(float* p32, void* p16, float* g32, const float* lr_ptr, float grad_scale,
                       int64_t n, int sm_count, cudaStream_t stream);
void launch_cast_pad(const float* src, int src_cols, void* dst, int dst_cols, int64_t rows,
                     cudaStream_t stream);

bool launch_gemm_tn_fused(const void* A, int64_t lda, const void* B, int64_t ldb, const void* bias,
                          void* C, int64_t ldc, int M, int N, int K, int epi, const void* act,
                          int64_t ldact, float* colsum, int block_n, int sm_count,
                          cudaStream_t stream);
bool launch_gemm_tn_bias_act(const void* A, int64_t lda, const void* B, int64_t ldb,
                             const void* bias, void* C, int64_t ldc, int M, int N, int K,
                             bool relu, int block_n, int sm_count, cudaStream_t stream);

}
```

distributed_embeddings_b200/ops/csrc/dense_kernels.cu:

```cuda
#include <cuda_bf16.h>
#include <cuda_runtime.h>
#include <stdint.h>

#include <cstdlib>

#include "common.cuh"
#include "de_b200.h"

namespace de {

namespace {

using bf16 = __nv_bfloat16;

__device__ __forceinline__ uint32_t smem_u32(const void* p) {
  return static_cast<uint32_t>(__cvta_generic_to_shared(p));
}

__device__ __forceinline__ void ldmatrix_x4(uint32_t (&r)[4], uint32_t addr) {
  asm volatile("ldmatrix.sync.aligned.m8n8.x4.shared.b16 {%0,%1,%2,%3}, [%4];"
               : "=r"(r[0]), "=r"(r[1]), "=r"(r[2]), "=r"(r[3])
               : "r"(addr));
}
__device__ __forceinline__ void ldmatrix_x4_trans(uint32_t (&r)[4], uint32_t addr) {
  asm volatile("ldmatrix.sync.aligned.m8n8.x4.trans.shared.b16 {%0,%1,%2,%3}, [%4];"
               : "=r"(r[0]), "=r"(r[1]), "=r"(r[2]), "=r"(r[3])
               : "r"(addr));
}
__device__ __forceinline__ void mma_bf16(float (&c)[4], const uint32_t (&a)[4], uint32_t b0,
                                         uint32_t b1) {
  asm volatile(
      "mma.sync.aligned.m16n8k16.row.col.f32.bf16.bf16.f32 {%0,%1,%2,%3}, {%4,%5,%6,%7}, "
      "{%8,%9}, {%0,%1,%2,%3};"
      : "+f"(c[0]), "+f"(c[1]), "+f"(c[2]), "+f"(c[3])
      : "r"(a[0]), "r"(a[1]), "r"(a[2]), "r"(a[3]), "r"(b0), "r"(b1));
}

constexpr int kMaxFeat = 32;
constexpr int kWarps = 4;

__host__ __device__ constexpr int fwd_warp_bytes(int d) {
  return (kMaxFeat * (d + 8) * 2 > kMaxFeat * 33 * 4) ? kMaxFeat * (d + 8) * 2 : kMaxFeat * 33 * 4;
}

__device__ __forceinline__ void cp_async16(void* smem_dst, const void* gmem_src) {
  asm volatile("cp.async.cg.shared.global [%0], [%1], 16;" ::"r"(smem_u32(smem_dst)),
               "l"(gmem_src)
               : "memory");
}
__device__ __forceinline__ void cp_async_wait_all() {
  asm volatile("cp.async.commit_group;\ncp.async.wait_group 0;" ::: "memory");
}

template <int D>
__device__ __forceinline__ void stage_features(bf16* sF, int LD, const bf16* bottom,
                                               const bf16* emb, int n_emb, int lane) {
  constexpr int kChunks = D / 8;
  const int total = (n_emb + 1) * kChunks;
#pragma unroll 4
  for (int c = lane; c < total; c += 32) {
    const int row = c / kChunks, ch = c - row * kChunks;
    const bf16* src = row == 0 ? bottom + ch * 8 : emb + (row - 1) * D + ch * 8;
    cp_async16(sF + row * LD + ch * 8, src);
  }
  cp_async_wait_all();
}

template <int D>
__device__ __forceinline__ void zero_pad_rows(bf16* sF, int LD, int n_emb, int lane) {
  constexpr int kChunks = D / 8;
  for (int c = (n_emb + 1) * kChunks + lane; c < kMaxFeat * kChunks; c += 32) {
    const int row = c / kChunks, ch = c - row * kChunks;
    *reinterpret_cast<uint4*>(sF + row * LD + ch * 8) = make_uint4(0, 0, 0, 0);
  }
}

template <int D>
__global__ void __launch_bounds__(kWarps * 32)
interact_fwd_kernel(const bf16* __restrict__ bottom, int64_t bottom_stride,
                    const bf16* __restrict__ emb, int64_t emb_stride, int n_emb,
                    bf16* __restrict__ z, int64_t z_stride, int z_width, int64_t batch,
                    const __grid_constant__ SyncArgs sync) {
  sync_head(sync);
  constexpr int LD = D + 8;
  constexpr int kWarpBytes = fwd_warp_bytes(D);
  extern __shared__ __align__(16) unsigned char smem_raw[];
  const int warp = threadIdx.x >> 5, lane = threadIdx.x & 31;
  bf16* sF = reinterpret_cast<bf16*>(smem_raw + warp * kWarpBytes);
  float* sC = reinterpret_cast<float*>(sF);
  const int nf = n_emb + 1;
  const int n_inter = nf * (nf - 1) / 2;

  for (int64_t s = static_cast<int64_t>(blockIdx.x) * kWarps + warp; s < batch;
       s += static_cast<int64_t>(gridDim.x) * kWarps) {
    const bf16* bp = bottom + s * bottom_stride;
    zero_pad_rows<D>(sF, LD, n_emb, lane);
    stage_features<D>(sF, LD, bp, emb + s * emb_stride, n_emb, lane);
    __syncwarp();
    float acc0[2][4] = {}, acc1[4][4] = {};
#pragma unroll
    for (int k = 0; k < D; k += 16) {
      uint32_t a0[4], a1[4], b01[4], b23[4];
      const int arow = lane & 15, acol = k + ((lane >> 4) << 3);
      ldmatrix_x4(a0, smem_u32(sF + arow * LD + acol));
      ldmatrix_x4(a1, smem_u32(sF + (16 + arow) * LD + acol));
      const int brow = (lane & 7) + ((lane >> 4) << 3), bcol = k + (((lane >> 3) & 1) << 3);
      ldmatrix_x4(b01, smem_u32(sF + brow * LD + bcol));
      ldmatrix_x4(b23, smem_u32(sF + (16 + brow) * LD + bcol));
      mma_bf16(acc0[0], a0, b01[0], b01[1]);
      mma_bf16(acc0[1], a0, b01[2], b01[3]);
      mma_bf16(acc1[0], a1, b01[0], b01[1]);
      mma_bf16(acc1[1], a1, b01[2], b01[3]);
      mma_bf16(acc1[2], a1, b23[0], b23[1]);
      mma_bf16(acc1[3], a1, b23[2], b23[3]);
    }
    __syncwarp();
    const int cr = lane >> 2, cc = (lane & 3) << 1;
#pragma unroll
    for (int nt = 0; nt < 2; ++nt) {
      sC[cr * 33 + nt * 8 + cc] = acc0[nt][0];
      sC[cr * 33 + nt * 8 + cc + 1] = acc0[nt][1];
      sC[(cr + 8) * 33 + nt * 8 + cc] = acc0[nt][2];
      sC[(cr + 8) * 33 + nt * 8 + cc + 1] = acc0[nt][3];
    }
#pragma unroll
    for (int nt = 0; nt < 4; ++nt) {
      sC[(16 + cr) * 33 + nt * 8 + cc] = acc1[nt][0];
      sC[(16 + cr) * 33 + nt * 8 + cc + 1] = acc1[nt][1];
      sC[(24 + cr) * 33 + nt * 8 + cc] = acc1[nt][2];
      sC[(24 + cr) * 33 + nt * 8 + cc + 1] = acc1[nt][3];
    }
    __syncwarp();
    bf16* zp = z + s * z_stride;
    for (int idx = lane; idx < n_inter; idx += 32) {
      int i = static_cast<int>((1.0f + sqrtf(1.0f + 8.0f * idx)) * 0.5f);
      while (i * (i - 1) / 2 > idx) --i;
      while ((i + 1) * i / 2 <= idx) ++i;
      const int j = idx - i * (i - 1) / 2;
      zp[idx] = __float2bfloat16_rn(sC[i * 33 + j]);
    }
    for (int c = lane; c < D; c += 32) zp[n_inter + c] = bp[c];
    for (int c = n_inter + D + lane; c < z_width; c += 32) zp[c] = __float2bfloat16_rn(0.f);
    __syncwarp();
  }
  sync_tail(sync);
}

template <int D>
__global__ void __launch_bounds__(kWarps * 32)
interact_bwd_kernel(const bf16* __restrict__ bottom, int64_t bottom_stride,
                    const bf16* __restrict__ emb, int64_t emb_stride, int n_emb,
                    const bf16* __restrict__ dz, int64_t dz_stride, bf16* __restrict__ dbottom,
                    int64_t dbottom_stride, bf16* __restrict__ demb, int64_t demb_stride,
                    float emb_grad_scale, int64_t batch) {
  constexpr int LD = D + 8;
  constexpr int LDG = 40;
  extern __shared__ __align__(16) unsigned char smem_raw[];
  const int warp = threadIdx.x >> 5, lane = threadIdx.x & 31;
  bf16* sF = reinterpret_cast<bf16*>(smem_raw) + warp * (kMaxFeat * LD + kMaxFeat * LDG);
  bf16* sG = sF + kMaxFeat * LD;
  const int nf = n_emb + 1;
  const int n_inter = nf * (nf - 1) / 2;
  zero_pad_rows<D>(sF, LD, n_emb, lane);

  for (int64_t s = static_cast<int64_t>(blockIdx.x) * kWarps + warp; s < batch;
       s += static_cast<int64_t>(gridDim.x) * kWarps) {
    stage_features<D>(sF, LD, bottom + s * bottom_stride, emb + s * emb_stride, n_emb, lane);
    const bf16* dzp = dz + s * dz_stride;
    for (int c = lane; c < kMaxFeat * LDG / 8; c += 32)
      reinterpret_cast<uint4*>(sG)[c] = make_uint4(0, 0, 0, 0);
    __syncwarp();
    for (int idx = lane; idx < n_inter; idx += 32) {
      int i = static_cast<int>((1.0f + sqrtf(1.0f + 8.0f * idx)) * 0.5f);
      while (i * (i - 1) / 2 > idx) --i;
      while ((i + 1) * i / 2 <= idx) ++i;
      const int j = idx - i * (i - 1) / 2;
      const bf16 v = dzp[idx];
      sG[i * LDG + j] = v;
      sG[j * LDG + i] = v;
    }
    __syncwarp();
    uint32_t ga[2][2][4];
#pragma unroll
    for (int mt = 0; mt < 2; ++mt)
#pragma unroll
      for (int ks = 0; ks < 2; ++ks)
        ldmatrix_x4(ga[mt][ks],
                    smem_u32(sG + (mt * 16 + (lane & 15)) * LDG + ks * 16 + ((lane >> 4) << 3)));
    const int cr = lane >> 2, cc = (lane & 3) << 1;
    bf16* dbp = dbottom + s * dbottom_stride;
    bf16* dep = demb + s * demb_stride;
#pragma unroll 1
    for (int n0 = 0; n0 < D; n0 += 32) {
      float acc[2][4][4] = {};
#pragma unroll
      for (int ks = 0; ks < 2; ++ks) {
        uint32_t b01[4], b23[4];
        const int krow = ks * 16 + (lane & 7) + (((lane >> 3) & 1) << 3);
        const int ncol = n0 + ((lane >> 4) << 3);
        ldmatrix_x4_trans(b01, smem_u32(sF + krow * LD + ncol));
        ldmatrix_x4_trans(b23, smem_u32(sF + krow * LD + ncol + 16));
#pragma unroll
        for (int mt = 0; mt < 2; ++mt) {
          mma_bf16(acc[mt][0], ga[mt][ks], b01[0], b01[1]);
          mma_bf16(acc[mt][1], ga[mt][ks], b01[2], b01[3]);
          mma_bf16(acc[mt][2], ga[mt][ks], b23[0], b23[1]);
          mma_bf16(acc[mt][3], ga[mt][ks], b23[2], b23[3]);
        }
      }
#pragma unroll
      for (int mt = 0; mt < 2; ++mt) {
#pragma unroll
        for (int nt = 0; nt < 4; ++nt) {
#pragma unroll
          for (int half = 0; half < 2; ++half) {
            const int row = mt * 16 + cr + half * 8;
            const int col = n0 + nt * 8 + cc;
            float v0 = acc[mt][nt][half * 2], v1 = acc[mt][nt][half * 2 + 1];
            if (row == 0) {
              v0 += __bfloat162float(dzp[n_inter + col]);
              v1 += __bfloat162float(dzp[n_inter + col + 1]);
              *reinterpret_cast<__nv_bfloat162*>(dbp + col) = __floats2bfloat162_rn(v0, v1);
            } else if (row <= n_emb) {
              *reinterpret_cast<__nv_bfloat162*>(dep + (row - 1) * D + col) =
                  __floats2bfloat162_rn(v0 * emb_grad_scale, v1 * emb_grad_scale);
            }
          }
        }
      }
    }
    __syncwarp();
  }
}

__device__ __forceinline__ void cp_async_commit() {
  asm volatile("cp.async.commit_group;" ::: "memory");
}
template <int N>
__device__ __forceinline__ void cp_async_wait_group() {
  asm volatile("cp.async.wait_group %0;" ::"n"(N) : "memory");
}

constexpr int kDzMax = 512;

template <int D>
__device__ __forceinline__ void issue_sample(bf16* sF, int LD, bf16* sDz, const bf16* bottom,
                                             const bf16* emb, const bf16* dz, int n_emb,
                                             int dz_chunks, int lane) {
  constexpr int kChunks = D / 8;
  const int total = (n_emb + 1) * kChunks;
#pragma unroll 4
  for (int c = lane; c < total; c += 32) {
    const int row = c / kChunks, ch = c - row * kChunks;
    const bf16* src = row == 0 ? bottom + ch * 8 : emb + (row - 1) * D + ch * 8;
    cp_async16(sF + row * LD + ch * 8, src);
  }
  for (int c = lane; c < dz_chunks; c += 32) cp_async16(sDz + c * 8, dz + c * 8);
}

struct ChunkDst {
  unsigned long long base;
  long long stride;
};

template <int D>
__global__ void __launch_bounds__(kWarps * 32)
interact_bwd_v2_kernel(const bf16* __restrict__ bottom, int64_t bottom_stride,
                       const bf16* __restrict__ emb, int64_t emb_stride, int n_emb,
                       const bf16* __restrict__ dz, int64_t dz_stride, bf16* __restrict__ dbottom,
                       int64_t dbottom_stride, bf16* __restrict__ demb, int64_t demb_stride,
                       float emb_grad_scale, int64_t batch,
                       const GradRoute* __restrict__ routes, int n_routes,
                       const __grid_constant__ SyncArgs sync, uint32_t* __restrict__ done_counters,
                       int chunk_rows) {
  constexpr int LD = D + 8;
  constexpr int LDG = 40;
  constexpr int kWarpElems = 2 * kMaxFeat * LD + 2 * kDzMax + kMaxFeat * LDG;
  constexpr int kRowChunks = D / 8;
  extern __shared__ __align__(16) unsigned char smem_raw[];
  const int warp = threadIdx.x >> 5, lane = threadIdx.x & 31;
  bf16* base = reinterpret_cast<bf16*>(smem_raw) + warp * kWarpElems;
  bf16* sDz0 = base + 2 * kMaxFeat * LD;
  bf16* sG = sDz0 + 2 * kDzMax;
  ChunkDst* sDst = reinterpret_cast<ChunkDst*>(reinterpret_cast<bf16*>(smem_raw) +
                                               kWarps * kWarpElems);
  const int nf = n_emb + 1;
  const int n_inter = nf * (nf - 1) / 2;
  const int dz_chunks = (n_inter + D + 7) >> 3;
  const int n_chunks = n_emb * kRowChunks;
  if (routes == nullptr) {
    for (int c = threadIdx.x; c < n_chunks; c += blockDim.x) {
      sDst[c].base = reinterpret_cast<unsigned long long>(demb + c * 8);
      sDst[c].stride = demb_stride * 2;
    }
  } else {
    for (int r = 0; r < n_routes; ++r) {
      const GradRoute R = routes[r];
      const int c0 = R.src_col >> 3, nc = R.width >> 3;
      for (int c = threadIdx.x; c < nc; c += blockDim.x) {
        sDst[c0 + c].base =
            reinterpret_cast<unsigned long long>(reinterpret_cast<bf16*>(R.dst) + R.dst_col + c * 8);
        sDst[c0 + c].stride = R.dst_stride * 2;
      }
    }
  }
  zero_pad_rows<D>(base, LD, n_emb, lane);
  zero_pad_rows<D>(base + kMaxFeat * LD, LD, n_emb, lane);
  __syncthreads();

  const int64_t stride = static_cast<int64_t>(gridDim.x) * kWarps;
  int64_t s = static_cast<int64_t>(blockIdx.x) * kWarps + warp;
  int cur = 0;
  if (s < batch)
    issue_sample<D>(base, LD, sDz0, bottom + s * bottom_stride, emb + s * emb_stride,
                    dz + s * dz_stride, n_emb, dz_chunks, lane);
  cp_async_commit();
  for (; s < batch; s += stride, cur ^= 1) {
    const int64_t nxt = s + stride;
    if (nxt < batch)
      issue_sample<D>(base + (cur ^ 1) * (kMaxFeat * LD), LD, sDz0 + (cur ^ 1) * kDzMax,
                      bottom + nxt * bottom_stride, emb + nxt * emb_stride, dz + nxt * dz_stride,
                      n_emb, dz_chunks, lane);
    cp_async_commit();
    cp_async_wait_group<1>();
    __syncwarp();
    bf16* sF = base + cur * (kMaxFeat * LD);
    const bf16* sDz = sDz0 + cur * kDzMax;
    for (int c = lane; c < kMaxFeat * LDG / 8; c += 32)
      reinterpret_cast<uint4*>(sG)[c] = make_uint4(0, 0, 0, 0);
    __syncwarp();
    for (int idx = lane; idx < n_inter; idx += 32) {
      int i = static_cast<int>((1.0f + sqrtf(1.0f + 8.0f * idx)) * 0.5f);
      while (i * (i - 1) / 2 > idx) --i;
      while ((i + 1) * i / 2 <= idx) ++i;
      const int j = idx - i * (i - 1) / 2;
      const bf16 v = sDz[idx];
      sG[i * LDG + j] = v;
      sG[j * LDG + i] = v;
    }
    __syncwarp();
    uint32_t ga[2][2][4];
#pragma unroll
    for (int mt = 0; mt < 2; ++mt)
#pragma unroll
      for (int ks = 0; ks < 2; ++ks)
        ldmatrix_x4(ga[mt][ks],
                    smem_u32(sG + (mt * 16 + (lane & 15)) * LDG + ks * 16 + ((lane >> 4) << 3)));
    const int cr = lane >> 2, cc = (lane & 3) << 1;
#pragma unroll 1
    for (int n0 = 0; n0 < D; n0 += 32) {
      float acc[2][4][4] = {};
#pragma unroll
      for (int ks = 0; ks < 2; ++ks) {
        uint32_t b01[4], b23[4];
        const int krow = ks * 16 + (lane & 7) + (((lane >> 3) & 1) << 3);
        const int ncol = n0 + ((lane >> 4) << 3);
        ldmatrix_x4_trans(b01, smem_u32(sF + krow * LD + ncol));
        ldmatrix_x4_trans(b23, smem_u32(sF + krow * LD + ncol + 16));
#pragma unroll
        for (int mt = 0; mt < 2; ++mt) {
          mma_bf16(acc[mt][0], ga[mt][ks], b01[0], b01[1]);
          mma_bf16(acc[mt][1], ga[mt][ks], b01[2], b01[3]);
          mma_bf16(acc[mt][2], ga[mt][ks], b23[0], b23[1]);
          mma_bf16(acc[mt][3], ga[mt][ks], b23[2], b23[3]);
        }
      }
#pragma unroll
      for (int mt = 0; mt < 2; ++mt) {
#pragma unroll
        for (int nt = 0; nt < 4; ++nt) {
#pragma unroll
          for (int half = 0; half < 2; ++half) {
            const int row = mt * 16 + cr + half * 8;
            const int col = n0 + nt * 8 + cc;
            float v0 = acc[mt][nt][half * 2], v1 = acc[mt][nt][half * 2 + 1];
            if (row == 0) {
              v0 += __bfloat162float(sDz[n_inter + col]);
              v1 += __bfloat162float(sDz[n_inter + col + 1]);
            } else {
              v0 *= emb_grad_scale;
              v1 *= emb_grad_scale;
            }
            if (row <= n_emb)
              *reinterpret_cast<__nv_bfloat162*>(sF + row * LD + col) =
                  __floats2bfloat162_rn(v0, v1);
          }
        }
      }
    }
    __syncwarp();
    if (lane < kRowChunks)
      *reinterpret_cast<uint4*>(dbottom + s * dbottom_stride + lane * 8) =
          *reinterpret_cast<const uint4*>(sF + lane * 8);
    for (int c = lane; c < n_chunks; c += 32) {
      const int row = 1 + c / kRowChunks, ch = c - (row - 1) * kRowChunks;
      const ChunkDst d = sDst[c];
      *reinterpret_cast<uint4*>(d.base + static_cast<unsigned long long>(s * d.stride)) =
          *reinterpret_cast<const uint4*>(sF + row * LD + ch * 8);
    }
    __syncwarp();
    if (done_counters != nullptr && lane == 0) {
      __threadfence();
      atomicAdd(done_counters + s / chunk_rows, 1u);
    }
  }
  cp_async_wait_group<0>();
  sync_tail(sync);
}

constexpr int kRbUnroll = 4;
__global__ void __launch_bounds__(256)
relu_bwd_bias_kernel(bf16* __restrict__ dy, const bf16* __restrict__ y, float* __restrict__ db,
                     int64_t rows, int cols, int rows_per_block) {
  extern __shared__ float s_part[];
  const int tpr = cols >> 3;
  const int rows_par = blockDim.x / tpr;
  const int tr = threadIdx.x / tpr, tc = threadIdx.x - tr * tpr;
  const int64_t r0 = static_cast<int64_t>(blockIdx.x) * rows_per_block;
  const int64_t r1 = min(rows, r0 + rows_per_block);
  float acc[8] = {0, 0, 0, 0, 0, 0, 0, 0};
  if (tr < rows_par) {
    for (int64_t r = r0 + tr; r < r1; r += static_cast<int64_t>(rows_par) * kRbUnroll) {
      uint4 g[kRbUnroll], a[kRbUnroll];
#pragma unroll
      for (int u = 0; u < kRbUnroll; ++u) {
        const int64_t rr = r + static_cast<int64_t>(u) * rows_par;
        if (rr < r1) {
          g[u] = *reinterpret_cast<const uint4*>(dy + rr * cols + tc * 8);
          a[u] = *reinterpret_cast<const uint4*>(y + rr * cols + tc * 8);
        }
      }
#pragma unroll
      for (int u = 0; u < kRbUnroll; ++u) {
        const int64_t rr = r + static_cast<int64_t>(u) * rows_par;
        if (rr < r1) {
          uint32_t* gw = reinterpret_cast<uint32_t*>(&g[u]);
          const uint32_t* aw = reinterpret_cast<const uint32_t*>(&a[u]);
#pragma unroll
          for (int i = 0; i < 4; ++i) {
            float2 gf = __bfloat1622float2(*reinterpret_cast<__nv_bfloat162*>(&gw[i]));
            const float2 af = __bfloat1622float2(*reinterpret_cast<const __nv_bfloat162*>(&aw[i]));
            gf.x = af.x > 0.f ? gf.x : 0.f;
            gf.y = af.y > 0.f ? gf.y : 0.f;
            acc[2 * i] += gf.x;
            acc[2 * i + 1] += gf.y;
            __nv_bfloat162 h = __floats2bfloat162_rn(gf.x, gf.y);
            gw[i] = *reinterpret_cast<uint32_t*>(&h);
          }
          *reinterpret_cast<uint4*>(dy + rr * cols + tc * 8) = g[u];
        }
      }
    }
#pragma unroll
    for (int i = 0; i < 8; ++i) s_part[tr * cols + tc * 8 + i] = acc[i];
  }
  __syncthreads();
  for (int c = threadIdx.x; c < cols; c += blockDim.x) {
    float v = 0.f;
    for (int t = 0; t < rows_par; ++t) v += s_part[t * cols + c];
    atomicAdd(db + c, v);
  }
}

template <int PL>
__global__ void __launch_bounds__(256)
head_loss_kernel(const bf16* __restrict__ x, int K, const bf16* __restrict__ w,
                 const bf16* __restrict__ bias, const float* __restrict__ labels, int64_t batch,
                 float inv_batch, bf16* __restrict__ dx, float* __restrict__ dw,
                 float* __restrict__ db, float* __restrict__ dbias_prev,
                 float* __restrict__ loss_sum, float* __restrict__ logits_out) {
  extern __shared__ float sred[];
  float* s_dw = sred;
  float* s_dbp = sred + K;
  float* s_misc = sred + 2 * K;
  for (int i = threadIdx.x; i < 2 * K + 2; i += blockDim.x) sred[i] = 0.f;
  __syncthreads();
  const int warp = threadIdx.x >> 5, lane = threadIdx.x & 31;
  const int wpb = blockDim.x >> 5;
  constexpr int per_lane = PL;
  const float b0 = __bfloat162float(bias[0]);
  float wreg[PL];
#pragma unroll
  for (int i = 0; i < PL; ++i) wreg[i] = __bfloat162float(w[lane + 32 * i]);
  float dw_acc[PL], dbp_acc[PL];
#pragma unroll
  for (int i = 0; i < PL; ++i) dw_acc[i] = dbp_acc[i] = 0.f;
  float loss_acc = 0.f, db_acc = 0.f;
  for (int64_t s = static_cast<int64_t>(blockIdx.x) * wpb + warp; s < batch;
       s += static_cast<int64_t>(gridDim.x) * wpb) {
    float xv[PL];
    float dot = 0.f;
#pragma unroll
    for (int i = 0; i < PL; ++i) {
      if (i < per_lane) {
        xv[i] = __bfloat162float(x[s * K + lane + 32 * i]);
        dot = fmaf(xv[i], wreg[i], dot);
      }
    }
#pragma unroll
    for (int off = 16; off > 0; off >>= 1) dot += __shfl_xor_sync(0xffffffffu, dot, off);
    const float logit = dot + b0;
    const float label = labels[s];
    const float loss = fmaxf(logit, 0.f) - logit * label + log1pf(__expf(-fabsf(logit)));
    const float sig = 1.f / (1.f + __expf(-logit));
    const float dl = (sig - label) * inv_batch;
    if (lane == 0) {
      loss_acc += loss;
      db_acc += dl;
      if (logits_out) logits_out[s] = logit;
    }
#pragma unroll
    for (int i = 0; i < PL; ++i) {
      if (i < per_lane) {
        dw_acc[i] = fmaf(dl, xv[i], dw_acc[i]);
        const float g = xv[i] > 0.f ? dl * wreg[i] : 0.f;
        dbp_acc[i] += g;
        dx[s * K + lane + 32 * i] = __float2bfloat16_rn(g);
      }
    }
  }
#pragma unroll
  for (int i = 0; i < PL; ++i) {
    if (i < per_lane) {
      atomicAdd(&s_dw[lane + 32 * i], dw_acc[i]);
      atomicAdd(&s_dbp[lane + 32 * i], dbp_acc[i]);
    }
  }
  if (lane == 0) {
    atomicAdd(&s_misc[0], loss_acc);
    atomicAdd(&s_misc[1], db_acc);
  }
  __syncthreads();
  for (int i = threadIdx.x; i < K; i += blockDim.x) {
    atomicAdd(dw + i, s_dw[i]);
    atomicAdd(dbias_prev + i, s_dbp[i]);
  }
  if (threadIdx.x == 0) {
    atomicAdd(loss_sum, s_misc[0] * inv_batch);
    atomicAdd(db, s_misc[1]);
  }
}

__global__ void __launch_bounds__(256)
sgd_update_kernel(float* __restrict__ p32, bf16* __restrict__ p16, float* __restrict__ g32,
                  const float* __restrict__ lr_ptr, float grad_scale, int64_t n_vec4) {
  const float step = -(*lr_ptr) * grad_scale;
  const int64_t stride = static_cast<int64_t>(gridDim.x) * blockDim.x;
  for (int64_t i = static_cast<int64_t>(blockIdx.x) * blockDim.x + threadIdx.x; i < n_vec4;
       i += stride) {
    float4 p = reinterpret_cast<float4*>(p32)[i];
    const float4 g = reinterpret_cast<const float4*>(g32)[i];
    p.x = fmaf(step, g.x, p.x);
    p.y = fmaf(step, g.y, p.y);
    p.z = fmaf(step, g.z, p.z);
    p.w = fmaf(step, g.w, p.w);
    reinterpret_cast<float4*>(p32)[i] = p;
    reinterpret_cast<float4*>(g32)[i] = make_float4(0.f, 0.f, 0.f, 0.f);
    __nv_bfloat162 a = __floats2bfloat162_rn(p.x, p.y), b = __floats2bfloat162_rn(p.z, p.w);
    uint2 o;
    o.x = *reinterpret_cast<uint32_t*>(&a);
    o.y = *reinterpret_cast<uint32_t*>(&b);
    reinterpret_cast<uint2*>(p16)[i] = o;
  }
}

__global__ void cast_pad_kernel(const float* __restrict__ src, int src_cols, bf16* __restrict__ dst,
                                int dst_cols, int64_t rows) {
  const int64_t n = rows * dst_cols;
  const int64_t stride = static_cast<int64_t>(gridDim.x) * blockDim.x;
  for (int64_t i = static_cast<int64_t>(blockIdx.x) * blockDim.x + threadIdx.x; i < n;
       i += stride) {
    const int64_t r = i / dst_cols;
    const int c = static_cast<int>(i - r * dst_cols);
    dst[i] = __float2bfloat16_rn(c < src_cols ? src[r * src_cols + c] : 0.f);
  }
}

__global__ void __launch_bounds__(256)
avgpool_fwd_kernel(const bf16* __restrict__ x, int64_t x_stride, int n, bf16* __restrict__ out,
                   int64_t out_stride, int out_len, int stride, int left, int64_t rows) {
  const int64_t total = rows * out_len;
  const int64_t step = static_cast<int64_t>(gridDim.x) * blockDim.x;
  for (int64_t i = static_cast<int64_t>(blockIdx.x) * blockDim.x + threadIdx.x; i < total;
       i += step) {
    const int64_t r = i / out_len;
    const int j = static_cast<int>(i - r * out_len);
    const int lo = max(0, j * stride - left), hi = min(n, (j + 1) * stride - left);
    const bf16* xp = x + r * x_stride;
    float acc = 0.f;
    for (int c = lo; c < hi; ++c) acc += __bfloat162float(xp[c]);
    out[r * out_stride + j] = __float2bfloat16_rn(hi > lo ? acc / static_cast<float>(hi - lo) : 0.f);
  }
}

__global__ void __launch_bounds__(256)
avgpool_bwd_kernel(const bf16* __restrict__ dout, int64_t dout_stride, int out_len,
                   bf16* __restrict__ dx, int64_t dx_stride, int n, int stride, int left,
                   int64_t rows) {
  const int64_t total = rows * n;
  const int64_t step = static_cast<int64_t>(gridDim.x) * blockDim.x;
  for (int64_t i = static_cast<int64_t>(blockIdx.x) * blockDim.x + threadIdx.x; i < total;
       i += step) {
    const int64_t r = i / n;
    const int c = static_cast<int>(i - r * n);
    const int j = (c + left) / stride;
    const int lo = max(0, j * stride - left), hi = min(n, (j + 1) * stride - left);
    const float g = j < out_len ? __bfloat162float(dout[r * dout_stride + j]) : 0.f;
    dx[r * dx_stride + c] = __float2bfloat16_rn(g / static_cast<float>(hi - lo));
  }
}

}

void launch_avgpool_fwd(const void* x, int64_t x_stride, int n, void* out, int64_t out_stride,
                        int out_len, int stride, int left, int64_t rows, cudaStream_t stream) {
  if (rows <= 0 || out_len <= 0) return;
  int64_t blocks = (rows * out_len + 255) / 256;
  if (blocks > kGridCapSms * 16) blocks = kGridCapSms * 16;
  avgpool_fwd_kernel<<<static_cast<unsigned>(blocks), 256, 0, stream>>>(
      reinterpret_cast<const bf16*>(x), x_stride, n, reinterpret_cast<bf16*>(out), out_stride,
      out_len, stride, left, rows);
}

void launch_avgpool_bwd(const void* dout, int64_t dout_stride, int out_len, void* dx,
                        int64_t dx_stride, int n, int stride, int left, int64_t rows,
                        cudaStream_t stream) {
  if (rows <= 0 || n <= 0) return;
  int64_t blocks = (rows * n + 255) / 256;
  if (blocks > kGridCapSms * 16) blocks = kGridCapSms * 16;
  avgpool_bwd_kernel<<<static_cast<unsigned>(blocks), 256, 0, stream>>>(
      reinterpret_cast<const bf16*>(dout), dout_stride, out_len, reinterpret_cast<bf16*>(dx),
      dx_stride, n, stride, left, rows);
}

bool launch_interact_fwd(const void* bottom, int64_t bottom_stride, const void* emb,
                         int64_t emb_stride, int n_emb, int dim, void* z, int64_t z_stride,
                         int z_width, int64_t batch, int sm_count, cudaStream_t stream,
                         const SyncArgs& sync) {
  if (n_emb + 1 > kMaxFeat || batch <= 0) return false;
  int64_t blocks = (batch + kWarps - 1) / kWarps;
  const int64_t cap = static_cast<int64_t>(sm_count) * 8;
  if (blocks > cap) blocks = cap;
#define DE_IFWD(DD)                                                                              \
  {                                                                                              \
    const size_t smem = kWarps * fwd_warp_bytes(DD);                                             \
    cudaFuncSetAttribute(interact_fwd_kernel<DD>, cudaFuncAttributeMaxDynamicSharedMemorySize,   \
                         static_cast<int>(smem));                                                \
    interact_fwd_kernel<DD><<<static_cast<unsigned>(blocks), kWarps * 32, smem, stream>>>(       \
        reinterpret_cast<const bf16*>(bottom), bottom_stride, reinterpret_cast<const bf16*>(emb), \
        emb_stride, n_emb, reinterpret_cast<bf16*>(z), z_stride, z_width, batch, sync);          \
    return true;                                                                                 \
  }
  if (dim == 128) DE_IFWD(128)
  if (dim == 64) DE_IFWD(64)
  if (dim == 32) DE_IFWD(32)
  if (dim == 16) DE_IFWD(16)
#undef DE_IFWD
  return false;
}

bool launch_interact_bwd(const void* bottom, int64_t bottom_stride, const void* emb,
                         int64_t emb_stride, int n_emb, int dim, const void* dz,
                         int64_t dz_stride, void* dbottom, int64_t dbottom_stride, void* demb,
                         int64_t demb_stride, float emb_grad_scale, int64_t batch, int sm_count,
                         cudaStream_t stream, const GradRoute* routes, int n_routes,
                         const SyncArgs& sync, uint32_t* done_counters, int chunk_rows) {
  if (n_emb + 1 > kMaxFeat || batch <= 0 || dim % 32 != 0) return false;
  int64_t blocks = (batch + kWarps - 1) / kWarps;
  const int64_t cap = static_cast<int64_t>(sm_count) * 8;
  if (blocks > cap) blocks = cap;
  static const bool force_v1 = [] {
    const char* v = std::getenv("DE_B200_INTERACT_V1");
    return v != nullptr && v[0] == '1';
  }();
  const int nf = n_emb + 1;
  const int dz_elems = (nf * (nf - 1) / 2 + dim + 7) / 8 * 8;
  const bool v2_ok =
      dz_elems <= kDzMax && dz_elems <= dz_stride && dz_stride % 8 == 0 &&
      bottom_stride % 8 == 0 && emb_stride % 8 == 0 && dbottom_stride % 8 == 0 &&
      ((reinterpret_cast<uintptr_t>(dz) | reinterpret_cast<uintptr_t>(bottom) |
        reinterpret_cast<uintptr_t>(emb) | reinterpret_cast<uintptr_t>(dbottom)) & 15) == 0 &&
      (dim == 128 || dim == 64) &&
      (routes != nullptr || (demb_stride % 8 == 0 && (reinterpret_cast<uintptr_t>(demb) & 15) == 0));
  if ((routes != nullptr || done_counters != nullptr) && !v2_ok) return false;
  const bool has_sync = sync.state != nullptr && (sync.wait_ch >= 0 || sync.signal_ch >= 0);
  if (v2_ok && (!force_v1 || routes != nullptr || has_sync || done_counters != nullptr)) {
    int64_t blocks2 = (batch + kWarps - 1) / kWarps;
    if (blocks2 > static_cast<int64_t>(sm_count) * 2) blocks2 = static_cast<int64_t>(sm_count) * 2;
#define DE_IBWD2(DD)                                                                             \
  {                                                                                              \
    const size_t smem =                                                                          \
        kWarps * (2 * kMaxFeat * (DD + 8) + 2 * kDzMax + kMaxFeat * 40) * sizeof(bf16) +         \
        static_cast<size_t>(n_emb) * (DD / 8) * sizeof(ChunkDst);                                \
    cudaFuncSetAttribute(interact_bwd_v2_kernel<DD>,                                             \
                         cudaFuncAttributeMaxDynamicSharedMemorySize, static_cast<int>(smem));   \
    interact_bwd_v2_kernel<DD><<<static_cast<unsigned>(blocks2), kWarps * 32, smem, stream>>>(   \
        reinterpret_cast<const bf16*>(bottom), bottom_stride, reinterpret_cast<const bf16*>(emb), \
        emb_stride, n_emb, reinterpret_cast<const bf16*>(dz), dz_stride,                         \
        reinterpret_cast<bf16*>(dbottom), dbottom_stride, reinterpret_cast<bf16*>(demb),         \
        demb_stride, emb_grad_scale, batch, routes, n_routes, sync, done_counters, chunk_rows);  \
    return true;                                                                                 \
  }
    if (dim == 128) DE_IBWD2(128)
    if (dim == 64) DE_IBWD2(64)
#undef DE_IBWD2
  }
  if (has_sync) return false;
#define DE_IBWD(DD)                                                                              \
  {                                                                                              \
    const size_t smem = kWarps * (kMaxFeat * (DD + 8) + kMaxFeat * 40) * sizeof(bf16);           \
    cudaFuncSetAttribute(interact_bwd_kernel<DD>, cudaFuncAttributeMaxDynamicSharedMemorySize,   \
                         static_cast<int>(smem));                                                \
    interact_bwd_kernel<DD><<<static_cast<unsigned>(blocks), kWarps * 32, smem, stream>>>(       \
        reinterpret_cast<const bf16*>(bottom), bottom_stride, reinterpret_cast<const bf16*>(emb), \
        emb_stride, n_emb, reinterpret_cast<const bf16*>(dz), dz_stride,                         \
        reinterpret_cast<bf16*>(dbottom), dbottom_stride, reinterpret_cast<bf16*>(demb),         \
        demb_stride, emb_grad_scale, batch);                                                     \
    return true;                                                                                 \
  }
  if (dim == 128) DE_IBWD(128)
  if (dim == 64) DE_IBWD(64)
  if (dim == 32) DE_IBWD(32)
#undef DE_IBWD
  return false;
}

void launch_relu_bwd_bias(void* dy, const void* y, float* db, int64_t rows, int cols,
                          cudaStream_t stream) {
  if (rows <= 0) return;
  const int tpr = cols / 8;
  const int threads = 256;
  const int rows_par = threads / tpr;
  const int rows_per_block = rows_par * kRbUnroll * 4;
  const int64_t blocks = (rows + rows_per_block - 1) / rows_per_block;
  const size_t smem = static_cast<size_t>(rows_par) * cols * sizeof(float);
  relu_bwd_bias_kernel<<<static_cast<unsigned>(blocks), threads, smem, stream>>>(
      reinterpret_cast<bf16*>(dy), reinterpret_cast<const bf16*>(y), db, rows, cols,
      rows_per_block);
}

bool launch_head_loss(const void* x, int K, const void* w, const void* bias, const float* labels,
                      int64_t batch, float inv_batch, void* dx, float* dw, float* db,
                      float* dbias_prev, float* loss_sum, float* logits_out, int sm_count,
                      cudaStream_t stream) {
  if (batch <= 0) return true;
  const int threads = 256;
  int64_t blocks = (batch + 7) / 8;
  if (blocks > sm_count * 4) blocks = sm_count * 4;
  const size_t smem = (2 * K + 2) * sizeof(float);
#define DE_HEAD(PL)                                                                              \
  head_loss_kernel<PL><<<static_cast<unsigned>(blocks), threads, smem, stream>>>(                \
      reinterpret_cast<const bf16*>(x), K, reinterpret_cast<const bf16*>(w),                     \
      reinterpret_cast<const bf16*>(bias), labels, batch, inv_batch, reinterpret_cast<bf16*>(dx), \
      dw, db, dbias_prev, loss_sum, logits_out)
  switch (K) {
    case 64: DE_HEAD(2); break;
    case 128: DE_HEAD(4); break;
    case 256: DE_HEAD(8); break;
    case 512: DE_HEAD(16); break;
    case 1024: DE_HEAD(32); break;
    default: return false;
  }
#undef DE_HEAD
  return true;
}

void launch_sgd_update(float* p32, void* p16, float* g32, const float* lr_ptr, float grad_scale,
                       int64_t n, int sm_count, cudaStream_t stream) {
  const int64_t n_vec4 = n / 4;
  if (n_vec4 <= 0) return;
  int64_t blocks = (n_vec4 + 255) / 256;
  if (blocks > sm_count * 8) blocks = sm_count * 8;
  sgd_update_kernel<<<static_cast<unsigned>(blocks), 256, 0, stream>>>(
      p32, reinterpret_cast<bf16*>(p16), g32, lr_ptr, grad_scale, n_vec4);
}

void launch_cast_pad(const float* src, int src_cols, void* dst, int dst_cols, int64_t rows,
                     cudaStream_t stream) {
  if (rows <= 0) return;
  int64_t blocks = (rows * dst_cols + 255) / 256;
  if (blocks > kGridCapSms * 8) blocks = kGridCapSms * 8;
  cast_pad_kernel<<<static_cast<unsigned>(blocks), 256, 0, stream>>>(
      src, src_cols, reinterpret_cast<bf16*>(dst), dst_cols, rows);
}

}
```

Before: 14.73 million.

## Pipeline interaction kernels with multi-stage cp.async and fuse bottom ReLU-bias backward

The interaction forward and backward kernels now use a three-stage cp.async ring per warp, so loads for upcoming samples overlap compute on the current one. Block size is chosen at launch from the available shared memory and occupancy. The forward kernel builds each z row in shared memory and writes it out with vectorized stores, replacing per-element index math. The bottom-MLP ReLU backward and bias gradient is folded into interact_bwd, which removes a separate pass over dy, at the cost of more shared memory per warp and a more complex kernel.

Measured after the change: 15.08 million, median of 6. 1.02x the previous value.

```diff
diff --git a/distributed_embeddings_b200/models/dlrm_fast.py b/distributed_embeddings_b200/models/dlrm_fast.py
--- a/distributed_embeddings_b200/models/dlrm_fast.py
+++ b/distributed_embeddings_b200/models/dlrm_fast.py
@@ -256,13 +256,13 @@
       eng.push_counters.zero_()
       self._push_ready.record(torch.cuda.current_stream())
       ops.interact_bwd(hb.y, eng.out, self.n_emb, self.dz, hb.dy, 0, 0, 1.0, eng.routes_stage,
-                       len(eng.routes_stage_np), [], eng.push_counters, eng.push_chunk_rows)
+                       len(eng.routes_stage_np), [], eng.push_counters, eng.push_chunk_rows, hb.gb)
       self._push_stream.wait_event(self._push_ready)
       with torch.cuda.stream(self._push_stream):
         eng.launch_streamed_push()
     else:
       ops.interact_bwd(hb.y, eng.out, self.n_emb, self.dz, hb.dy, 0, 0, 1.0, eng.routes_all,
-                       len(eng.routes_all_np), eng.sync_grad_signal(), None, 0)
+                       len(eng.routes_all_np), eng.sync_grad_signal(), None, 0, hb.gb)
     if self._side is not None:
       self._side.wait_stream(torch.cuda.current_stream())
       if pushed:
@@ -273,7 +273,6 @@
       if pushed:
         torch.cuda.current_stream().wait_stream(self._push_stream)
       eng.backward_inplace()
-    ops.relu_bwd_bias(hb.dy, hb.y, hb.gb)
     for i in range(len(self.bottom) - 1, -1, -1):
       L = self.bottom[i]
       x = self.bottom[i - 1].y if i > 0 else self.x0
diff --git a/distributed_embeddings_b200/ops/csrc/bindings.cpp b/distributed_embeddings_b200/ops/csrc/bindings.cpp
--- a/distributed_embeddings_b200/ops/csrc/bindings.cpp
+++ b/distributed_embeddings_b200/ops/csrc/bindings.cpp
@@ -749,7 +749,8 @@
 void interact_bwd(const Tensor& bottom, const Tensor& emb, int64_t n_emb, const Tensor& dz,
                   Tensor dbottom, int64_t demb_ptr, int64_t demb_stride, double emb_grad_scale,
                   const c10::optional<Tensor>& routes, int64_t n_routes, at::IntArrayRef sync,
-                  const c10::optional<Tensor>& done_counters, int64_t chunk_rows) {
+                  const c10::optional<Tensor>& done_counters, int64_t chunk_rows,
+                  const c10::optional<Tensor>& gb) {
   check_bf16_2d(bottom, "bottom");
   check_bf16_2d(emb, "emb");
   check_bf16_2d(dz, "dz");
@@ -759,6 +760,10 @@
                 routes->numel() >= n_routes * static_cast<int64_t>(sizeof(de::GradRoute)));
   c10::cuda::CUDAGuard guard(bottom.device());
   const int64_t dim = bottom.size(1);
+  if (gb.has_value())
+    TORCH_CHECK(gb->is_cuda() && gb->scalar_type() == at::kFloat && gb->is_contiguous() &&
+                    gb->numel() >= dim,
+                "gb must be a contiguous fp32 CUDA tensor with at least dim entries");
   bool ok = de::launch_interact_bwd(bottom.data_ptr(), bottom.stride(0), emb.data_ptr(),
                                     emb.stride(0), static_cast<int>(n_emb), static_cast<int>(dim),
                                     dz.data_ptr(), dz.stride(0), dbottom.data_ptr(),
@@ -772,7 +777,8 @@
                                     done_counters.has_value()
                                         ? reinterpret_cast<uint32_t*>(done_counters->data_ptr<int>())
                                         : nullptr,
-                                    static_cast<int>(chunk_rows));
+                                    static_cast<int>(chunk_rows),
+                                    gb.has_value() ? gb->data_ptr<float>() : nullptr);
   TORCH_CHECK(ok, "unsupported interaction shape (n_emb <= 31, dim in {32,64,128}; routed / "
                   "signalling launches need dim in {64,128} and 16-byte aligned rows)");
   check_launch();
@@ -1040,7 +1046,7 @@
   m.def(
       "interact_bwd(Tensor bottom, Tensor emb, int n_emb, Tensor dz, Tensor(a!) dbottom, "
       "int demb_ptr, int demb_stride, float emb_grad_scale, Tensor? routes, int n_routes, "
-      "int[] sync, Tensor? done_counters, int chunk_rows) -> ()",
+      "int[] sync, Tensor? done_counters, int chunk_rows, Tensor(b!)? gb=None) -> ()",
       &interact_bwd);
   m.def("avgpool_fwd(Tensor x, int n, Tensor(a!) out, int stride) -> ()", &avgpool_fwd);
   m.def("avgpool_bwd(Tensor dout, Tensor(a!) dx, int n, int stride) -> ()", &avgpool_bwd);
diff --git a/distributed_embeddings_b200/ops/csrc/de_b200.h b/distributed_embeddings_b200/ops/csrc/de_b200.h
--- a/distributed_embeddings_b200/ops/csrc/de_b200.h
+++ b/distributed_embeddings_b200/ops/csrc/de_b200.h
@@ -191,7 +191,7 @@
                          int64_t demb_stride, float emb_grad_scale, int64_t batch, int sm_count,
                          cudaStream_t stream, const GradRoute* routes, int n_routes,
                          const SyncArgs& sync, uint32_t* done_counters = nullptr,
-                         int chunk_rows = 0);
+                         int chunk_rows = 0, float* gb = nullptr);
 void launch_avgpool_fwd(const void* x, int64_t x_stride, int n, void* out, int64_t out_stride,
                         int out_len, int stride, int left, int64_t rows, cudaStream_t stream);
 void launch_avgpool_bwd(const void* dout, int64_t dout_stride, int out_len, void* dx,
diff --git a/distributed_embeddings_b200/ops/csrc/dense_kernels.cu b/distributed_embeddings_b200/ops/csrc/dense_kernels.cu
--- a/distributed_embeddings_b200/ops/csrc/dense_kernels.cu
+++ b/distributed_embeddings_b200/ops/csrc/dense_kernels.cu
@@ -39,10 +39,6 @@
 constexpr int kMaxFeat = 32;
 constexpr int kWarps = 4;
 
-__host__ __device__ constexpr int fwd_warp_bytes(int d) {
-  return (kMaxFeat * (d + 8) * 2 > kMaxFeat * 33 * 4) ? kMaxFeat * (d + 8) * 2 : kMaxFeat * 33 * 4;
-}
-
 __device__ __forceinline__ void cp_async16(void* smem_dst, const void* gmem_src) {
   asm volatile("cp.async.cg.shared.global [%0], [%1], 16;" ::"r"(smem_u32(smem_dst)),
                "l"(gmem_src)
@@ -51,9 +47,16 @@
 __device__ __forceinline__ void cp_async_wait_all() {
   asm volatile("cp.async.commit_group;\ncp.async.wait_group 0;" ::: "memory");
 }
+__device__ __forceinline__ void cp_async_commit() {
+  asm volatile("cp.async.commit_group;" ::: "memory");
+}
+template <int N>
+__device__ __forceinline__ void cp_async_wait_group() {
+  asm volatile("cp.async.wait_group %0;" ::"n"(N) : "memory");
+}
 
 template <int D>
-__device__ __forceinline__ void stage_features(bf16* sF, int LD, const bf16* bottom,
+__device__ __forceinline__ void issue_features(bf16* sF, int LD, const bf16* bottom,
                                                const bf16* emb, int n_emb, int lane) {
   constexpr int kChunks = D / 8;
   const int total = (n_emb + 1) * kChunks;
@@ -63,6 +66,12 @@
     const bf16* src = row == 0 ? bottom + ch * 8 : emb + (row - 1) * D + ch * 8;
     cp_async16(sF + row * LD + ch * 8, src);
   }
+}
+
+template <int D>
+__device__ __forceinline__ void stage_features(bf16* sF, int LD, const bf16* bottom,
+                                               const bf16* emb, int n_emb, int lane) {
+  issue_features<D>(sF, LD, bottom, emb, n_emb, lane);
   cp_async_wait_all();
 }
 
@@ -75,38 +84,79 @@
   }
 }
 
+constexpr int kStages = 3;
+constexpr int kMaxBlockWarps = 16;
+
+__host__ __device__ constexpr int round8(int n) { return (n + 7) & ~7; }
+
+template <int LD>
+__device__ __forceinline__ const bf16* feature_row(const bf16* sF, int r, int nf,
+                                                   const bf16* sZero) {
+  return r < nf ? sF + r * LD : sZero;
+}
+
+__host__ __device__ constexpr int fwd_warp_elems(int d, int n_emb) {
+  return kStages * (n_emb + 1) * (d + 8) + round8((n_emb + 1) * n_emb / 2 + d);
+}
+
 template <int D>
-__global__ void __launch_bounds__(kWarps * 32)
+__global__ void __launch_bounds__(kMaxBlockWarps * 32)
 interact_fwd_kernel(const bf16* __restrict__ bottom, int64_t bottom_stride,
                     const bf16* __restrict__ emb, int64_t emb_stride, int n_emb,
                     bf16* __restrict__ z, int64_t z_stride, int z_width, int64_t batch,
-                    const __grid_constant__ SyncArgs sync) {
+                    bool z_vec, const __grid_constant__ SyncArgs sync) {
   sync_head(sync);
   constexpr int LD = D + 8;
-  constexpr int kWarpBytes = fwd_warp_bytes(D);
   extern __shared__ __align__(16) unsigned char smem_raw[];
-  const int warp = threadIdx.x >> 5, lane = threadIdx.x & 31;
-  bf16* sF = reinterpret_cast<bf16*>(smem_raw + warp * kWarpBytes);
-  float* sC = reinterpret_cast<float*>(sF);
+  const int warp = threadIdx.x >> 5, lane = threadIdx.x & 31, n_warps = blockDim.x >> 5;
   const int nf = n_emb + 1;
   const int n_inter = nf * (nf - 1) / 2;
-
-  for (int64_t s = static_cast<int64_t>(blockIdx.x) * kWarps + warp; s < batch;
-       s += static_cast<int64_t>(gridDim.x) * kWarps) {
-    const bf16* bp = bottom + s * bottom_stride;
-    zero_pad_rows<D>(sF, LD, n_emb, lane);
-    stage_features<D>(sF, LD, bp, emb + s * emb_stride, n_emb, lane);
+  const int stage_elems = nf * LD;
+  const int zrow = round8(n_inter + D);
+  bf16* sZero = reinterpret_cast<bf16*>(smem_raw);
+  bf16* sF0 = sZero + LD + warp * fwd_warp_elems(D, n_emb);
+  bf16* sZ = sF0 + kStages * stage_elems;
+  for (int c = threadIdx.x; c < LD / 8; c += blockDim.x)
+    reinterpret_cast<uint4*>(sZero)[c] = make_uint4(0, 0, 0, 0);
+  for (int c = n_inter + D + lane; c < zrow; c += 32) sZ[c] = __float2bfloat16_rn(0.f);
+
+  const int64_t stride = static_cast<int64_t>(gridDim.x) * n_warps;
+  const int64_t s0 = static_cast<int64_t>(blockIdx.x) * n_warps + warp;
+#pragma unroll
+  for (int k = 0; k < kStages - 1; ++k) {
+    const int64_t t = s0 + k * stride;
+    if (t < batch)
+      issue_features<D>(sF0 + k * stage_elems, LD, bottom + t * bottom_stride,
+                        emb + t * emb_stride, n_emb, lane);
+    cp_async_commit();
+  }
+  __syncthreads();
+  const int cr = lane >> 2, cc = (lane & 3) << 1;
+  int st = 0;
+  for (int64_t s = s0; s < batch; s += stride) {
+    const int64_t t = s + (kStages - 1) * stride;
+    const int st_fill = st == 0 ? kStages - 1 : st - 1;
+    if (t < batch)
+      issue_features<D>(sF0 + st_fill * stage_elems, LD, bottom + t * bottom_stride,
+                        emb + t * emb_stride, n_emb, lane);
+    cp_async_commit();
+    cp_async_wait_group<kStages - 1>();
     __syncwarp();
+    const bf16* sF = sF0 + st * stage_elems;
+    const int arow = lane & 15, brow = (lane & 7) + ((lane >> 4) << 3);
+    const bf16* pa0 = feature_row<LD>(sF, arow, nf, sZero);
+    const bf16* pa1 = feature_row<LD>(sF, 16 + arow, nf, sZero);
+    const bf16* pb0 = feature_row<LD>(sF, brow, nf, sZero);
+    const bf16* pb1 = feature_row<LD>(sF, 16 + brow, nf, sZero);
     float acc0[2][4] = {}, acc1[4][4] = {};
 #pragma unroll
     for (int k = 0; k < D; k += 16) {
       uint32_t a0[4], a1[4], b01[4], b23[4];
-      const int arow = lane & 15, acol = k + ((lane >> 4) << 3);
-      ldmatrix_x4(a0, smem_u32(sF + arow * LD + acol));
-      ldmatrix_x4(a1, smem_u32(sF + (16 + arow) * LD + acol));
-      const int brow = (lane & 7) + ((lane >> 4) << 3), bcol = k + (((lane >> 3) & 1) << 3);
-      ldmatrix_x4(b01, smem_u32(sF + brow * LD + bcol));
-      ldmatrix_x4(b23, smem_u32(sF + (16 + brow) * LD + bcol));
+      const int acol = k + ((lane >> 4) << 3), bcol = k + (((lane >> 3) & 1) << 3);
+      ldmatrix_x4(a0, smem_u32(pa0 + acol));
+      ldmatrix_x4(a1, smem_u32(pa1 + acol));
+      ldmatrix_x4(b01, smem_u32(pb0 + bcol));
+      ldmatrix_x4(b23, smem_u32(pb1 + bcol));
       mma_bf16(acc0[0], a0, b01[0], b01[1]);
       mma_bf16(acc0[1], a0, b01[2], b01[3]);
       mma_bf16(acc1[0], a1, b01[0], b01[1]);
@@ -114,35 +164,38 @@
       mma_bf16(acc1[2], a1, b23[0], b23[1]);
       mma_bf16(acc1[3], a1, b23[2], b23[3]);
     }
-    __syncwarp();
-    const int cr = lane >> 2, cc = (lane & 3) << 1;
+    auto put = [&](int i, int j, float v) {
+      if (j < i && i < nf) sZ[i * (i - 1) / 2 + j] = __float2bfloat16_rn(v);
+    };
 #pragma unroll
     for (int nt = 0; nt < 2; ++nt) {
-      sC[cr * 33 + nt * 8 + cc] = acc0[nt][0];
-      sC[cr * 33 + nt * 8 + cc + 1] = acc0[nt][1];
-      sC[(cr + 8) * 33 + nt * 8 + cc] = acc0[nt][2];
-      sC[(cr + 8) * 33 + nt * 8 + cc + 1] = acc0[nt][3];
+      put(cr, nt * 8 + cc, acc0[nt][0]);
+      put(cr, nt * 8 + cc + 1, acc0[nt][1]);
+      put(cr + 8, nt * 8 + cc, acc0[nt][2]);
+      put(cr + 8, nt * 8 + cc + 1, acc0[nt][3]);
     }
 #pragma unroll
     for (int nt = 0; nt < 4; ++nt) {
-      sC[(16 + cr) * 33 + nt * 8 + cc] = acc1[nt][0];
-      sC[(16 + cr) * 33 + nt * 8 + cc + 1] = acc1[nt][1];
-      sC[(24 + cr) * 33 + nt * 8 + cc] = acc1[nt][2];
-      sC[(24 + cr) * 33 + nt * 8 + cc + 1] = acc1[nt][3];
-    }
+      put(16 + cr, nt * 8 + cc, acc1[nt][0]);
+      put(16 + cr, nt * 8 + cc + 1, acc1[nt][1]);
+      put(24 + cr, nt * 8 + cc, acc1[nt][2]);
+      put(24 + cr, nt * 8 + cc + 1, acc1[nt][3]);
+    }
+    for (int c = lane; c < D; c += 32) sZ[n_inter + c] = sF[c];
     __syncwarp();
     bf16* zp = z + s * z_stride;
-    for (int idx = lane; idx < n_inter; idx += 32) {
-      int i = static_cast<int>((1.0f + sqrtf(1.0f + 8.0f * idx)) * 0.5f);
-      while (i * (i - 1) / 2 > idx) --i;
-      while ((i + 1) * i / 2 <= idx) ++i;
-      const int j = idx - i * (i - 1) / 2;
-      zp[idx] = __float2bfloat16_rn(sC[i * 33 + j]);
-    }
-    for (int c = lane; c < D; c += 32) zp[n_inter + c] = bp[c];
-    for (int c = n_inter + D + lane; c < z_width; c += 32) zp[c] = __float2bfloat16_rn(0.f);
+    if (z_vec) {
+      for (int c = lane; c < (z_width >> 3); c += 32)
+        *reinterpret_cast<uint4*>(zp + c * 8) =
+            c * 8 < zrow ? *reinterpret_cast<const uint4*>(sZ + c * 8) : make_uint4(0, 0, 0, 0);
+    } else {
+      for (int c = lane; c < z_width; c += 32)
+        zp[c] = c < n_inter + D ? sZ[c] : __float2bfloat16_rn(0.f);
+    }
     __syncwarp();
-  }
+    st = st + 1 == kStages ? 0 : st + 1;
+  }
+  cp_async_wait_group<0>();
   sync_tail(sync);
 }
 
@@ -233,28 +286,11 @@
   }
 }
 
-__device__ __forceinline__ void cp_async_commit() {
-  asm volatile("cp.async.commit_group;" ::: "memory");
-}
-template <int N>
-__device__ __forceinline__ void cp_async_wait_group() {
-  asm volatile("cp.async.wait_group %0;" ::"n"(N) : "memory");
-}
-
-constexpr int kDzMax = 512;
-
 template <int D>
 __device__ __forceinline__ void issue_sample(bf16* sF, int LD, bf16* sDz, const bf16* bottom,
                                              const bf16* emb, const bf16* dz, int n_emb,
                                              int dz_chunks, int lane) {
-  constexpr int kChunks = D / 8;
-  const int total = (n_emb + 1) * kChunks;
-#pragma unroll 4
-  for (int c = lane; c < total; c += 32) {
-    const int row = c / kChunks, ch = c - row * kChunks;
-    const bf16* src = row == 0 ? bottom + ch * 8 : emb + (row - 1) * D + ch * 8;
-    cp_async16(sF + row * LD + ch * 8, src);
-  }
+  issue_features<D>(sF, LD, bottom, emb, n_emb, lane);
   for (int c = lane; c < dz_chunks; c += 32) cp_async16(sDz + c * 8, dz + c * 8);
 }
 
@@ -263,8 +299,20 @@
   long long stride;
 };
 
+__host__ __device__ constexpr int bwd_block_bytes(int d, int n_emb) {
+  return n_emb * (d / 8) * static_cast<int>(sizeof(ChunkDst)) +
+         round8((n_emb + 1) * n_emb / 2) * 2 + (d + 8) * 2;
+}
+__host__ __device__ constexpr int bwd_stage_elems(int d, int n_emb) {
+  return (n_emb + 1) * (d + 8) + round8((n_emb + 1) * n_emb / 2 + d);
+}
+constexpr int kLDG = 40;
+__host__ __device__ constexpr int bwd_warp_elems(int d, int n_emb) {
+  return kStages * bwd_stage_elems(d, n_emb) + kMaxFeat * kLDG + d;
+}
+
 template <int D>
-__global__ void __launch_bounds__(kWarps * 32)
+__global__ void __launch_bounds__(kMaxBlockWarps * 32)
 interact_bwd_v2_kernel(const bf16* __restrict__ bottom, int64_t bottom_stride,
                        const bf16* __restrict__ emb, int64_t emb_stride, int n_emb,
                        const bf16* __restrict__ dz, int64_t dz_stride, bf16* __restrict__ dbottom,
@@ -272,22 +320,23 @@
                        float emb_grad_scale, int64_t batch,
                        const GradRoute* __restrict__ routes, int n_routes,
                        const __grid_constant__ SyncArgs sync, uint32_t* __restrict__ done_counters,
-                       int chunk_rows) {
+                       int chunk_rows, float* __restrict__ gb) {
   constexpr int LD = D + 8;
-  constexpr int LDG = 40;
-  constexpr int kWarpElems = 2 * kMaxFeat * LD + 2 * kDzMax + kMaxFeat * LDG;
   constexpr int kRowChunks = D / 8;
   extern __shared__ __align__(16) unsigned char smem_raw[];
-  const int warp = threadIdx.x >> 5, lane = threadIdx.x & 31;
-  bf16* base = reinterpret_cast<bf16*>(smem_raw) + warp * kWarpElems;
-  bf16* sDz0 = base + 2 * kMaxFeat * LD;
-  bf16* sG = sDz0 + 2 * kDzMax;
-  ChunkDst* sDst = reinterpret_cast<ChunkDst*>(reinterpret_cast<bf16*>(smem_raw) +
-                                               kWarps * kWarpElems);
+  const int warp = threadIdx.x >> 5, lane = threadIdx.x & 31, n_warps = blockDim.x >> 5;
   const int nf = n_emb + 1;
   const int n_inter = nf * (nf - 1) / 2;
   const int dz_chunks = (n_inter + D + 7) >> 3;
   const int n_chunks = n_emb * kRowChunks;
+  const int f_elems = nf * LD, stage_elems = bwd_stage_elems(D, n_emb);
+  ChunkDst* sDst = reinterpret_cast<ChunkDst*>(smem_raw);
+  uint16_t* sIJ = reinterpret_cast<uint16_t*>(sDst + n_chunks);
+  bf16* sZero = reinterpret_cast<bf16*>(sIJ + round8(n_inter));
+  bf16* base0 = sZero + LD;
+  bf16* base = base0 + warp * bwd_warp_elems(D, n_emb);
+  bf16* sG = base + kStages * stage_elems;
+  bf16* sDb = sG + kMaxFeat * kLDG;
   if (routes == nullptr) {
     for (int c = threadIdx.x; c < n_chunks; c += blockDim.x) {
       sDst[c].base = reinterpret_cast<unsigned long long>(demb + c * 8);
@@ -304,39 +353,50 @@
       }
     }
   }
-  zero_pad_rows<D>(base, LD, n_emb, lane);
-  zero_pad_rows<D>(base + kMaxFeat * LD, LD, n_emb, lane);
+  for (int idx = threadIdx.x; idx < n_inter; idx += blockDim.x) {
+    int i = static_cast<int>((1.0f + sqrtf(1.0f + 8.0f * idx)) * 0.5f);
+    while (i * (i - 1) / 2 > idx) --i;
+    while ((i + 1) * i / 2 <= idx) ++i;
+    sIJ[idx] = static_cast<uint16_t>(i | ((idx - i * (i - 1) / 2) << 8));
+  }
+  for (int c = threadIdx.x; c < LD / 8; c += blockDim.x)
+    reinterpret_cast<uint4*>(sZero)[c] = make_uint4(0, 0, 0, 0);
+  for (int c = lane; c < kMaxFeat * kLDG / 8; c += 32)
+    reinterpret_cast<uint4*>(sG)[c] = make_uint4(0, 0, 0, 0);
+
+  const int64_t stride = static_cast<int64_t>(gridDim.x) * n_warps;
+  const int64_t s0 = static_cast<int64_t>(blockIdx.x) * n_warps + warp;
+#pragma unroll
+  for (int k = 0; k < kStages - 1; ++k) {
+    const int64_t t = s0 + k * stride;
+    if (t < batch)
+      issue_sample<D>(base + k * stage_elems, LD, base + k * stage_elems + f_elems,
+                      bottom + t * bottom_stride, emb + t * emb_stride, dz + t * dz_stride, n_emb,
+                      dz_chunks, lane);
+    cp_async_commit();
+  }
   __syncthreads();
-
-  const int64_t stride = static_cast<int64_t>(gridDim.x) * kWarps;
-  int64_t s = static_cast<int64_t>(blockIdx.x) * kWarps + warp;
-  int cur = 0;
-  if (s < batch)
-    issue_sample<D>(base, LD, sDz0, bottom + s * bottom_stride, emb + s * emb_stride,
-                    dz + s * dz_stride, n_emb, dz_chunks, lane);
-  cp_async_commit();
-  for (; s < batch; s += stride, cur ^= 1) {
-    const int64_t nxt = s + stride;
-    if (nxt < batch)
-      issue_sample<D>(base + (cur ^ 1) * (kMaxFeat * LD), LD, sDz0 + (cur ^ 1) * kDzMax,
-                      bottom + nxt * bottom_stride, emb + nxt * emb_stride, dz + nxt * dz_stride,
-                      n_emb, dz_chunks, lane);
+  float gb_acc[8] = {0.f, 0.f, 0.f, 0.f, 0.f, 0.f, 0.f, 0.f};
+  const int cr = lane >> 2, cc = (lane & 3) << 1;
+  int st = 0;
+  for (int64_t s = s0; s < batch; s += stride) {
+    const int64_t t = s + (kStages - 1) * stride;
+    const int st_fill = st == 0 ? kStages - 1 : st - 1;
+    if (t < batch)
+      issue_sample<D>(base + st_fill * stage_elems, LD, base + st_fill * stage_elems + f_elems,
+                      bottom + t * bottom_stride, emb + t * emb_stride, dz + t * dz_stride, n_emb,
+                      dz_chunks, lane);
     cp_async_commit();
-    cp_async_wait_group<1>();
+    cp_async_wait_group<kStages - 1>();
     __syncwarp();
-    bf16* sF = base + cur * (kMaxFeat * LD);
-    const bf16* sDz = sDz0 + cur * kDzMax;
-    for (int c = lane; c < kMaxFeat * LDG / 8; c += 32)
-      reinterpret_cast<uint4*>(sG)[c] = make_uint4(0, 0, 0, 0);
-    __syncwarp();
+    bf16* sF = base + st * stage_elems;
+    const bf16* sDz = sF + f_elems;
     for (int idx = lane; idx < n_inter; idx += 32) {
-      int i = static_cast<int>((1.0f + sqrtf(1.0f + 8.0f * idx)) * 0.5f);
-      while (i * (i - 1) / 2 > idx) --i;
-      while ((i + 1) * i / 2 <= idx) ++i;
-      const int j = idx - i * (i - 1) / 2;
+      const uint32_t ij = sIJ[idx];
+      const int i = ij & 255, j = ij >> 8;
       const bf16 v = sDz[idx];
-      sG[i * LDG + j] = v;
-      sG[j * LDG + i] = v;
+      sG[i * kLDG + j] = v;
+      sG[j * kLDG + i] = v;
     }
     __syncwarp();
     uint32_t ga[2][2][4];
@@ -345,18 +405,19 @@
 #pragma unroll
       for (int ks = 0; ks < 2; ++ks)
         ldmatrix_x4(ga[mt][ks],
-                    smem_u32(sG + (mt * 16 + (lane & 15)) * LDG + ks * 16 + ((lane >> 4) << 3)));
-    const int cr = lane >> 2, cc = (lane & 3) << 1;
+                    smem_u32(sG + (mt * 16 + (lane & 15)) * kLDG + ks * 16 + ((lane >> 4) << 3)));
+    const int krow = (lane & 7) + (((lane >> 3) & 1) << 3);
+    const bf16* pk0 = feature_row<LD>(sF, krow, nf, sZero);
+    const bf16* pk1 = feature_row<LD>(sF, 16 + krow, nf, sZero);
 #pragma unroll 1
     for (int n0 = 0; n0 < D; n0 += 32) {
       float acc[2][4][4] = {};
 #pragma unroll
       for (int ks = 0; ks < 2; ++ks) {
         uint32_t b01[4], b23[4];
-        const int krow = ks * 16 + (lane & 7) + (((lane >> 3) & 1) << 3);
-        const int ncol = n0 + ((lane >> 4) << 3);
-        ldmatrix_x4_trans(b01, smem_u32(sF + krow * LD + ncol));
-        ldmatrix_x4_trans(b23, smem_u32(sF + krow * LD + ncol + 16));
+        const bf16* pk = (ks == 0 ? pk0 : pk1) + n0 + ((lane >> 4) << 3);
+        ldmatrix_x4_trans(b01, smem_u32(pk));
+        ldmatrix_x4_trans(b23, smem_u32(pk + 16));
 #pragma unroll
         for (int mt = 0; mt < 2; ++mt) {
           mma_bf16(acc[mt][0], ga[mt][ks], b01[0], b01[1]);
@@ -377,21 +438,36 @@
             if (row == 0) {
               v0 += __bfloat162float(sDz[n_inter + col]);
               v1 += __bfloat162float(sDz[n_inter + col + 1]);
-            } else {
-              v0 *= emb_grad_scale;
-              v1 *= emb_grad_scale;
+              *reinterpret_cast<__nv_bfloat162*>(sDb + col) = __floats2bfloat162_rn(v0, v1);
+            } else if (row <= n_emb) {
+              *reinterpret_cast<__nv_bfloat162*>(sF + row * LD + col) =
+                  __floats2bfloat162_rn(v0 * emb_grad_scale, v1 * emb_grad_scale);
             }
-            if (row <= n_emb)
-              *reinterpret_cast<__nv_bfloat162*>(sF + row * LD + col) =
-                  __floats2bfloat162_rn(v0, v1);
           }
         }
       }
     }
     __syncwarp();
-    if (lane < kRowChunks)
-      *reinterpret_cast<uint4*>(dbottom + s * dbottom_stride + lane * 8) =
-          *reinterpret_cast<const uint4*>(sF + lane * 8);
+    if (lane < kRowChunks) {
+      uint4 g = *reinterpret_cast<const uint4*>(sDb + lane * 8);
+      if (gb != nullptr) {
+        const uint4 y = *reinterpret_cast<const uint4*>(sF + lane * 8);
+        uint32_t* gw = reinterpret_cast<uint32_t*>(&g);
+        const uint32_t* yw = reinterpret_cast<const uint32_t*>(&y);
+#pragma unroll
+        for (int i = 0; i < 4; ++i) {
+          float2 gf = __bfloat1622float2(*reinterpret_cast<const __nv_bfloat162*>(&gw[i]));
+          const float2 yf = __bfloat1622float2(*reinterpret_cast<const __nv_bfloat162*>(&yw[i]));
+          gf.x = yf.x > 0.f ? gf.x : 0.f;
+          gf.y = yf.y > 0.f ? gf.y : 0.f;
+          gb_acc[2 * i] += gf.x;
+          gb_acc[2 * i + 1] += gf.y;
+          const __nv_bfloat162 h = __floats2bfloat162_rn(gf.x, gf.y);
+          gw[i] = *reinterpret_cast<const uint32_t*>(&h);
+        }
+      }
+      *reinterpret_cast<uint4*>(dbottom + s * dbottom_stride + lane * 8) = g;
+    }
     for (int c = lane; c < n_chunks; c += 32) {
       const int row = 1 + c / kRowChunks, ch = c - (row - 1) * kRowChunks;
       const ChunkDst d = sDst[c];
@@ -403,8 +479,21 @@
       __threadfence();
       atomicAdd(done_counters + s / chunk_rows, 1u);
     }
+    st = st + 1 == kStages ? 0 : st + 1;
   }
   cp_async_wait_group<0>();
+  if (gb != nullptr) {
+    if (lane < kRowChunks)
+#pragma unroll
+      for (int i = 0; i < 8; ++i) reinterpret_cast<float*>(base)[lane * 8 + i] = gb_acc[i];
+    __syncthreads();
+    for (int c = threadIdx.x; c < D; c += blockDim.x) {
+      float v = 0.f;
+      for (int w = 0; w < n_warps; ++w)
+        v += reinterpret_cast<const float*>(base0 + w * bwd_warp_elems(D, n_emb))[c];
+      atomicAdd(gb + c, v);
+    }
+  }
   sync_tail(sync);
 }
 
@@ -633,22 +722,57 @@
       dx_stride, n, stride, left, rows);
 }
 
+namespace {
+
+struct PipelinedShape {
+  int warps;
+  size_t smem;
+  unsigned blocks;
+};
+template <typename Kernel>
+bool pipelined_shape(Kernel kernel, size_t fixed, size_t per_warp, int64_t batch, int sm_count,
+                     PipelinedShape* out) {
+  int dev = 0, optin = 0;
+  cudaGetDevice(&dev);
+  cudaDeviceGetAttribute(&optin, cudaDevAttrMaxSharedMemoryPerBlockOptin, dev);
+  cudaFuncAttributes fa{};
+  cudaFuncGetAttributes(&fa, kernel);
+  const size_t avail = static_cast<size_t>(optin) - fa.sharedSizeBytes;
+  if (avail < fixed + per_warp) return false;
+  int warps = static_cast<int>((avail - fixed) / per_warp);
+  if (warps > kMaxBlockWarps) warps = kMaxBlockWarps;
+  const size_t smem = fixed + static_cast<size_t>(warps) * per_warp;
+  cudaFuncSetAttribute(kernel, cudaFuncAttributeMaxDynamicSharedMemorySize, static_cast<int>(smem));
+  int occ = 0;
+  cudaOccupancyMaxActiveBlocksPerMultiprocessor(&occ, kernel, warps * 32, smem);
+  if (occ < 1) occ = 1;
+  int64_t blocks = (batch + warps - 1) / warps;
+  if (blocks > static_cast<int64_t>(occ) * sm_count) blocks = static_cast<int64_t>(occ) * sm_count;
+  *out = {warps, smem, static_cast<unsigned>(blocks)};
+  return true;
+}
+
+bool aligned16(const void* p) { return (reinterpret_cast<uintptr_t>(p) & 15) == 0; }
+
+}
+
 bool launch_interact_fwd(const void* bottom, int64_t bottom_stride, const void* emb,
                          int64_t emb_stride, int n_emb, int dim, void* z, int64_t z_stride,
                          int z_width, int64_t batch, int sm_count, cudaStream_t stream,
                          const SyncArgs& sync) {
   if (n_emb + 1 > kMaxFeat || batch <= 0) return false;
-  int64_t blocks = (batch + kWarps - 1) / kWarps;
-  const int64_t cap = static_cast<int64_t>(sm_count) * 8;
-  if (blocks > cap) blocks = cap;
+  if (!aligned16(bottom) || !aligned16(emb) || bottom_stride % 8 != 0 || emb_stride % 8 != 0)
+    return false;
+  const bool z_vec = aligned16(z) && z_stride % 8 == 0 && z_width % 8 == 0;
 #define DE_IFWD(DD)                                                                              \
   {                                                                                              \
-    const size_t smem = kWarps * fwd_warp_bytes(DD);                                             \
-    cudaFuncSetAttribute(interact_fwd_kernel<DD>, cudaFuncAttributeMaxDynamicSharedMemorySize,   \
-                         static_cast<int>(smem));                                                \
-    interact_fwd_kernel<DD><<<static_cast<unsigned>(blocks), kWarps * 32, smem, stream>>>(       \
+    PipelinedShape sh;                                                                           \
+    if (!pipelined_shape(interact_fwd_kernel<DD>, (DD + 8) * sizeof(bf16),                       \
+                         fwd_warp_elems(DD, n_emb) * sizeof(bf16), batch, sm_count, &sh))        \
+      return false;                                                                              \
+    interact_fwd_kernel<DD><<<sh.blocks, sh.warps * 32, sh.smem, stream>>>(                      \
         reinterpret_cast<const bf16*>(bottom), bottom_stride, reinterpret_cast<const bf16*>(emb), \
-        emb_stride, n_emb, reinterpret_cast<bf16*>(z), z_stride, z_width, batch, sync);          \
+        emb_stride, n_emb, reinterpret_cast<bf16*>(z), z_stride, z_width, batch, z_vec, sync);   \
     return true;                                                                                 \
   }
   if (dim == 128) DE_IFWD(128)
@@ -664,7 +788,8 @@
                          int64_t dz_stride, void* dbottom, int64_t dbottom_stride, void* demb,
                          int64_t demb_stride, float emb_grad_scale, int64_t batch, int sm_count,
                          cudaStream_t stream, const GradRoute* routes, int n_routes,
-                         const SyncArgs& sync, uint32_t* done_counters, int chunk_rows) {
+                         const SyncArgs& sync, uint32_t* done_counters, int chunk_rows,
+                         float* gb) {
   if (n_emb + 1 > kMaxFeat || batch <= 0 || dim % 32 != 0) return false;
   int64_t blocks = (batch + kWarps - 1) / kWarps;
   const int64_t cap = static_cast<int64_t>(sm_count) * 8;
@@ -676,29 +801,25 @@
   const int nf = n_emb + 1;
   const int dz_elems = (nf * (nf - 1) / 2 + dim + 7) / 8 * 8;
   const bool v2_ok =
-      dz_elems <= kDzMax && dz_elems <= dz_stride && dz_stride % 8 == 0 &&
+      dz_elems <= dz_stride && dz_stride % 8 == 0 &&
       bottom_stride % 8 == 0 && emb_stride % 8 == 0 && dbottom_stride % 8 == 0 &&
-      ((reinterpret_cast<uintptr_t>(dz) | reinterpret_cast<uintptr_t>(bottom) |
-        reinterpret_cast<uintptr_t>(emb) | reinterpret_cast<uintptr_t>(dbottom)) & 15) == 0 &&
-      (dim == 128 || dim == 64) &&
-      (routes != nullptr || (demb_stride % 8 == 0 && (reinterpret_cast<uintptr_t>(demb) & 15) == 0));
+      aligned16(dz) && aligned16(bottom) && aligned16(emb) && aligned16(dbottom) &&
+      (dim == 128 || dim == 64) && (routes != nullptr || (demb_stride % 8 == 0 && aligned16(demb)));
   if ((routes != nullptr || done_counters != nullptr) && !v2_ok) return false;
   const bool has_sync = sync.state != nullptr && (sync.wait_ch >= 0 || sync.signal_ch >= 0);
   if (v2_ok && (!force_v1 || routes != nullptr || has_sync || done_counters != nullptr)) {
-    int64_t blocks2 = (batch + kWarps - 1) / kWarps;
-    if (blocks2 > static_cast<int64_t>(sm_count) * 2) blocks2 = static_cast<int64_t>(sm_count) * 2;
 #define DE_IBWD2(DD)                                                                             \
   {                                                                                              \
-    const size_t smem =                                                                          \
-        kWarps * (2 * kMaxFeat * (DD + 8) + 2 * kDzMax + kMaxFeat * 40) * sizeof(bf16) +         \
-        static_cast<size_t>(n_emb) * (DD / 8) * sizeof(ChunkDst);                                \
-    cudaFuncSetAttribute(interact_bwd_v2_kernel<DD>,                                             \
-                         cudaFuncAttributeMaxDynamicSharedMemorySize, static_cast<int>(smem));   \
-    interact_bwd_v2_kernel<DD><<<static_cast<unsigned>(blocks2), kWarps * 32, smem, stream>>>(   \
+    PipelinedShape sh;                                                                           \
+    if (!pipelined_shape(interact_bwd_v2_kernel<DD>, bwd_block_bytes(DD, n_emb),                 \
+                         bwd_warp_elems(DD, n_emb) * sizeof(bf16), batch, sm_count, &sh))        \
+      return false;                                                                              \
+    interact_bwd_v2_kernel<DD><<<sh.blocks, sh.warps * 32, sh.smem, stream>>>(                   \
         reinterpret_cast<const bf16*>(bottom), bottom_stride, reinterpret_cast<const bf16*>(emb), \
         emb_stride, n_emb, reinterpret_cast<const bf16*>(dz), dz_stride,                         \
         reinterpret_cast<bf16*>(dbottom), dbottom_stride, reinterpret_cast<bf16*>(demb),         \
-        demb_stride, emb_grad_scale, batch, routes, n_routes, sync, done_counters, chunk_rows);  \
+        demb_stride, emb_grad_scale, batch, routes, n_routes, sync, done_counters, chunk_rows,   \
+        gb);                                                                                     \
     return true;                                                                                 \
   }
     if (dim == 128) DE_IBWD2(128)
@@ -706,6 +827,7 @@
 #undef DE_IBWD2
   }
   if (has_sync) return false;
+  if (gb != nullptr && (bottom_stride != dim || dbottom_stride != dim)) return false;
 #define DE_IBWD(DD)                                                                              \
   {                                                                                              \
     const size_t smem = kWarps * (kMaxFeat * (DD + 8) + kMaxFeat * 40) * sizeof(bf16);           \
@@ -716,6 +838,7 @@
         emb_stride, n_emb, reinterpret_cast<const bf16*>(dz), dz_stride,                         \
         reinterpret_cast<bf16*>(dbottom), dbottom_stride, reinterpret_cast<bf16*>(demb),         \
         demb_stride, emb_grad_scale, batch);                                                     \
+    if (gb != nullptr) launch_relu_bwd_bias(dbottom, bottom, gb, batch, dim, stream);           \
     return true;                                                                                 \
   }
   if (dim == 128) DE_IBWD(128)
```
